# haliphinx/TCE-RVOS

Hardware: AMD Instinct MI355X
Metric: clips/s (T=5, 360×640, Swin-T) at 1/2/4/8 MI355X; mask IoU vs ref (higher is better)
Workload: dtype f32 (3xf16-split MFMA, f32 accumulate); 1 GPU; swin_t_p4w7 T=5 360x640 + 32-token text, B=1 clip per forward, flags --with_box_refine --binary --f_token 8 --qtrans (BASELINE config 2); clips_in_flight_per_gpu=1, clips_per_forward=1, same_clip_in_group=False, ranks_per_gpu=1, parallelism=clip-sharded x1

## Files before the change

include/tce_rvos.h:

```cpp
#ifndef TCE_RVOS_H
#define TCE_RVOS_H
#include <stdint.h>

#ifdef __cplusplus
extern "C" {
#endif

typedef void* tceStream;

int tce_abi_version(void);
const char* tce_last_error(void);

typedef struct {
  const float* A;
  const float* A2;
  const float* W;
  const float* bias;
  const float* res;
  float* C;
  int32_t M, N, K;
  int32_t lda, lda2, ldw, ldc, ldres;
  int32_t act, res_mode;
  int32_t batch;
  int64_t sA, sA2, sW, sBias, sC, sRes;
// ... 96 lines not shown
int tce_copy_segments(const tceCopySeg* segs, int32_t n, tceStream stream);
int tce_box_refine_f32(const float* tmp, const float* ref, float* out, int32_t n, int32_t ref_dim, tceStream stream);

int tce_mask_pack_f32(const float* params, float* w0f, float* tail, int32_t nl, int32_t T, int32_t Q, int32_t Cm,
                      tceStream stream);
int tce_mask_tail_f32(const float* G, const float* tail, const float* refs , int32_t ref_ld,
                      float* masks, int32_t nl, int32_t T, int32_t Q, int32_t h, int32_t w, float img_h, float img_w,
                      int32_t stride_px, tceStream stream);

int tce_select_masks_u8(const float* logits, const float* masks, uint8_t* out, int32_t* best_query, int32_t T,
                        int32_t Q, int32_t K, int32_t h, int32_t w, int32_t H0, int32_t W0, float threshold,
                        tceStream stream);

int tce_resize_h_u8(const uint8_t* in, const int32_t* coef, const int32_t* bounds, uint8_t* tmp, int64_t rows,
                    int32_t Win, int32_t Wout, int32_t ksize, tceStream stream);
int tce_resize_v_norm_f32(const uint8_t* tmp, const int32_t* coef, const int32_t* bounds, const float* lut, float* out,
                          int32_t T, int32_t Hin, int32_t W, int32_t Hout, int32_t ksize, tceStream stream);

int tce_embed_ln_f32(const int64_t* ids, const int64_t* pos_ids, const float* word, const float* pos, const float* type0,
                     const float* gamma, const float* beta, float* out, int32_t L, int32_t C, float eps, int32_t pad_id,
                     tceStream stream);
int tce_embed_ln_seqs_f32(const int64_t* ids, const float* word, const float* pos, const float* type0, const float* gamma,
                          const float* beta, float* out, int32_t nseq, int32_t seq_len, int32_t C, float eps, int32_t pad_id,
                          tceStream stream);
int tce_mha_small64_f32(const float* qkv, float* out, int32_t L, int32_t nheads, float scale, tceStream stream);
int tce_tanh_f32(const float* x, float* out, int64_t n, tceStream stream);

int32_t tce_thin_linear_splits(int32_t M, int32_t N, int32_t K);
int tce_thin_partials_f32(const float* x, int64_t ldx, int32_t xsplits, const float* bias_x, int32_t act_x, const float* W,
                          int64_t ldw, float* ws, int32_t M, int32_t N, int32_t K, tceStream stream);
int tce_splitk_reduce_f32(const float* ws, int32_t splits, int32_t M, int32_t N, const float* bias, int32_t act, const float* res,
                          int32_t ldres, int32_t res_mode, float* C, int32_t ldc, const float* gamma, const float* beta, float eps,
                          tceStream stream);
int tce_mha_small64_splits_f32(const float* qkv_planes, int32_t splits, const float* bias, float* out, int32_t L, int32_t nheads,
                               float scale, tceStream stream);
int tce_mha_small64_seqs_f32(const float* qkv_planes, int32_t splits, const float* bias, float* out, int32_t nseq, int32_t L,
                             int32_t nheads, float scale, tceStream stream);
int tce_mha_small64_lens_f32(const float* qkv_planes, int32_t splits, const float* bias, float* out, int32_t nseq, int32_t L,
                             int32_t nheads, float scale, const int32_t* lens, tceStream stream);
int tce_caption_lens_f32(const int64_t* ids, int32_t nseq, int32_t Lmax, int32_t pad_id, int32_t D, int32_t* lens, uint8_t* kmask,
                         float* pos, tceStream stream);

int64_t tce_ffn_packed_bytes(int32_t C, int32_t Hd);
int tce_ffn_pack_f32(const float* W1, const float* b1, const float* W2, void* packed, int32_t C, int32_t Hd,
                     tceStream stream);
int tce_ffn_pack_batched_f32(const float* W1, const float* b1, const float* W2, void* packed, int32_t C, int32_t Hd,
                             int32_t batch, tceStream stream);
int tce_ffn_fused_f32(const float* x, int64_t ldx, const void* packed, const float* b2, const float* g_in,
                      const float* be_in, float eps_in, const float* g_out, const float* be_out, float eps_out,
                      float* out, int64_t ldo, int32_t M, int32_t C, int32_t Hd, int32_t act, tceStream stream);
int64_t tce_ffn_split_ws_floats(int32_t M, int32_t C, int32_t Hd, int32_t act);
int32_t tce_ffn_split_counters(int32_t M, int32_t C, int32_t Hd, int32_t act);
int tce_ffn_fused_split_f32(const float* x, int64_t ldx, const void* packed, const float* b2, const float* g_in, const float* be_in,
                            float eps_in, const float* g_out, const float* be_out, float eps_out, float* out, int64_t ldo, int32_t M,
                            int32_t C, int32_t Hd, int32_t act, float* ws, int64_t ws_floats, int32_t* counters, int32_t n_counters,
                            tceStream stream);

typedef struct {
  const float* x;
  const float* a2;
  const void* packed;
  const float* bias;
  const float* res;
  float* out;
  const float *g_in, *be_in, *g_out, *be_out;
  int64_t ldx, lda2, ldres, ldo;
  int64_t sX, sA2, sRes, sOut;
  int32_t M, N, K, batch, a2_rows, act, res_mode;
  float eps_in, eps_out;
} tceRowLinArgs;
int64_t tce_rowlin_packed_bytes(int32_t N, int32_t K);
int tce_rowlin_pack_f32(const float* W, int64_t ldw, void* packed, int32_t N, int32_t K, tceStream stream);
int tce_rowlin_f32(const tceRowLinArgs* args, tceStream stream);

int64_t tce_conv3x3_packed_bytes(int32_t Cin, int32_t N);
int tce_conv3x3_pack_f32(const float* w, void* packed, int32_t Cin, int32_t N, tceStream stream);
int tce_conv3x3_f32(const float* x, int64_t ldx, const void* packed, const float* bias, float* out, int64_t ldo, int32_t T,
                    int32_t H, int32_t W, int32_t Cin, int32_t N, tceStream stream);
int64_t tce_conv3x3_split_ws_floats(int32_t M, int32_t Cin, int32_t N);
int32_t tce_conv3x3_split_pieces(int32_t M, int32_t Cin, int32_t N);
int32_t tce_conv3x3_split_kstep(int32_t pieces, int32_t s);
int tce_conv3x3_split_f32(const float* x, int64_t ldx, const void* packed, const float* bias, float* out, int64_t ldo, int32_t T,
                          int32_t H, int32_t W, int32_t Cin, int32_t N, float* ws, int64_t ws_floats, tceStream stream);

typedef struct {
  const float* x;
  const float* a2;
  const void* packed;
  const float* bo;
  const float* res;
  float* out;
  const float *g_out, *be_out;
  int64_t ldx, lda2, ldres, ldo;
  int64_t sX, sRes, sOut, sW;
  int32_t M, batch, a2_rows, res_mode, group;
  float eps_out;
  int32_t w_div;
} tceXattnArgs;
int tce_xattn_prepare_f32(const float* k, const float* v, const float* wqT_ext, const float* wo, float* W1, float* b1,
                          float* W2, int32_t L, int32_t group, int32_t batch, tceStream stream);
int tce_xattn_fused_f32(const tceXattnArgs* args, tceStream stream);

typedef struct {
  const void* packed;
  const float* b2;
  const float* g_out;
  const float* be_out;
  float* mid;
  int64_t ldmid, sMid;
  int32_t hidden, act;
  float eps_out;
} tceXattnFfnArgs;
int tce_ffn_pack_chain_f32(const float* W1, const float* b1, const float* W2, void* packed, int32_t C, int32_t Hd, tceStream stream);
int tce_xattn_ffn_fused_f32(const tceXattnArgs* args, const tceXattnFfnArgs* ffn, tceStream stream);
int tce_xattn_pack_f32(const float* k, const float* v, const float* wqT_ext, const float* wo, void* packed, int32_t L, int32_t group,
                       int32_t batch, tceStream stream);
int tce_xattn_prepare_lens_f32(const float* k, const float* v, const float* wqT_ext, const float* wo, float* W1, float* b1, float* W2,
                               int32_t L, int32_t group, int32_t batch, const int32_t* lens, tceStream stream);
int tce_xattn_pack_lens_f32(const float* k, const float* v, const float* wqT_ext, const float* wo, void* packed, int32_t L,
                            int32_t group, int32_t batch, const int32_t* lens, tceStream stream);

int64_t tce_swin_attn_packed_bytes(int32_t C);
int tce_swin_attn_pack_f32(const float* Wqkv, const float* Wproj, void* packed, int32_t C, tceStream stream);
int tce_swin_attn_fused_f32(const float* x, int64_t ldx, const void* packed, const float* qkv_bias, const float* proj_bias,
                            const float* bias_table, const float* gamma1, const float* beta1, float eps, float* out, int64_t ldo,
                            int32_t T, int32_t H, int32_t W, int32_t C, int32_t shift, tceStream stream);

int tce_graph_begin(tceStream stream);
int tce_graph_end(tceStream stream, void** graph_exec_out);
int tce_graph_launch(void* graph_exec, tceStream stream);
int tce_graph_destroy(void* graph_exec);
int tce_graph_group(void* const* graphs, int32_t n, void** graph_exec_out);

typedef struct {
  const float* W;
  const float* bias;
  float* out;
  int32_t N, ldw, ldo;
  int32_t use_a2;
  int32_t act;
} tceFewRowSeg;
typedef struct {
  const float* x;
  const float* a2;
  const float* res;
  int64_t ldx, lda2, ldres;
  int32_t a2_rows, R, K, nseg;
  tceFewRowSeg seg[3];
  const float* g_in;
  const float* be_in;
  float* xn_out;
  int64_t ldxn;
  float eps_in;
} tceFewRowArgs;
int tce_fewrow_linear_f32(const tceFewRowArgs* args, tceStream stream);

#ifdef __cplusplus
}
#endif
#endif
```

tce-rvos_amd/_lib.py:

```python
import ctypes as C
import os

HERE = os.path.dirname(os.path.abspath(__file__))
LIB_PATH = os.environ.get("TCE_LIB") or os.path.join(HERE, "lib", "libtce_rvos.so")

c_f = C.c_void_p
i32, i64, f32 = C.c_int32, C.c_int64, C.c_float


class GemmArgs(C.Structure):
    _fields_ = [("A", c_f), ("A2", c_f), ("W", c_f), ("bias", c_f), ("res", c_f), ("C", c_f),
                ("M", i32), ("N", i32), ("K", i32),
                ("lda", i32), ("lda2", i32), ("ldw", i32), ("ldc", i32), ("ldres", i32),
                ("act", i32), ("res_mode", i32), ("batch", i32),
                ("sA", i64), ("sA2", i64), ("sW", i64), ("sBias", i64), ("sC", i64), ("sRes", i64),
                ("conv", i32), ("T", i32), ("H", i32), ("Wd", i32), ("Cin", i32), ("Ho", i32), ("Wo", i32),
                ("kh", i32), ("kw", i32), ("stride", i32), ("pad", i32)]


class RowLinArgs(C.Structure):
    _fields_ = [("x", c_f), ("a2", c_f), ("packed", c_f), ("bias", c_f), ("res", c_f), ("out", c_f),
                ("g_in", c_f), ("be_in", c_f), ("g_out", c_f), ("be_out", c_f),
                ("ldx", i64), ("lda2", i64), ("ldres", i64), ("ldo", i64),
                ("sX", i64), ("sA2", i64), ("sRes", i64), ("sOut", i64),
# ... 29 lines not shown
class CopySeg(C.Structure):
    _fields_ = [("src", c_f), ("dst", c_f), ("rows", i64), ("row_words", i64), ("src_pitch_words", i64)]


SIGNATURES = {
    "tce_abi_version": (i32, []),
    "tce_last_error": (C.c_char_p, []),
    "tce_gemm_f32": (i32, [C.POINTER(GemmArgs), c_f]),
    "tce_gemm_splitk_f32": (i32, [C.POINTER(GemmArgs), i32, c_f, c_f]),
    "tce_gemm_splitk_ln_f32": (i32, [C.POINTER(GemmArgs), i32, c_f, c_f, c_f, f32, c_f]),
    "tce_gemm_select_tile": (i32, [i32, i32, i32]),
    "tce_gemm_select_tile_ex": (i32, [i32, i32, i32, i32, i32]),
    "tce_set_gemm_mode": (i32, [i32]),
    "tce_set_gemm_mode_thread": (i32, [i32]),
    "tce_set_range_flag": (i32, [c_f]),
    "tce_get_gemm_mode": (i32, []),
    "tce_layernorm_f32": (i32, [c_f, c_f, c_f, c_f, c_f, i64, i32, f32, c_f]),
    "tce_groupnorm_nsplit": (i32, [i32]),
    "tce_groupnorm_f32": (i32, [c_f, c_f, c_f, c_f, c_f, i32, i32, i32, i32, f32, i32, c_f]),
    "tce_groupnorm_up_add_f32": (i32, [c_f, c_f, c_f, c_f, c_f, c_f, i32, i32, i32, i32, i32, i32, i32, f32, i32, c_f]),
    "tce_resnet_stem_f32": (i32, [c_f, c_f, c_f, c_f, i32, i32, i32, c_f]),
    "tce_maxpool3x3s2_cl_f32": (i32, [c_f, c_f, i32, i32, i32, i32, c_f]),
    "tce_resize_h_u8": (i32, [c_f, c_f, c_f, c_f, i64, i32, i32, i32, c_f]),
    "tce_resize_v_norm_f32": (i32, [c_f, c_f, c_f, c_f, c_f, i32, i32, i32, i32, i32, c_f]),
    "tce_patch_embed_f32": (i32, [c_f, c_f, c_f, c_f, c_f, c_f, i32, i32, i32, i32, f32, c_f]),
    "tce_window_attn_f32": (i32, [c_f, c_f, c_f, c_f, i32, i32, i32, i32, i32, i32, c_f]),
    "tce_window_attn3d_f32": (i32, [c_f, c_f, c_f, c_f, i32, i32, i32, i32, i32, i32, c_f]),
    "tce_patch_merge_ln_f32": (i32, [c_f, c_f, c_f, c_f, i32, i32, i32, i32, f32, c_f]),
    "tce_mha_f32": (i32, [c_f, c_f, c_f, c_f, i32, i32, i32, i32, i32, i32, i32, i32, i64, i64, i64, i64, c_f, f32, c_f]),
    "tce_mha_ws_bytes": (i64, [i32, i32, i32]),
    "tce_mha_ws_f32": (i32, [c_f, c_f, c_f, c_f, c_f, i32, i32, i32, i32, i32, i32, i32, i32, i64, i64, i64, i64, c_f, f32, c_f]),
    "tce_ms_deform_attn_forward_f32": (i32, [c_f, c_f, c_f, c_f, c_f, c_f, i32, i32, i32, i32, i32, i32, i32, c_f]),
    "tce_ms_deform_attn_backward_f32": (i32, [c_f, c_f, c_f, c_f, c_f, c_f, c_f, c_f, c_f, i32, i32, i32, i32, i32, i32, i32, c_f]),
    "tce_msda_fused_f32": (i32, [c_f, c_f, c_f, c_f, C.POINTER(i32), i32, i32, i32, i32, i32, i32, i32, i32, c_f]),
    "tce_msda_fused_valid_f32": (i32, [c_f, c_f, c_f, c_f, C.POINTER(i32), C.POINTER(i32), i32, i32, i32, i32, i32, i32, i32,
                                       i32, c_f]),
    "tce_msda_fewq_raw_f32": (i32, [c_f, c_f, c_f, c_f, c_f, c_f, C.POINTER(i32), C.POINTER(i32), i32, i32, i32, i32, i32, i32, i32,
                                    i32, c_f]),
    "tce_contrastive_f32": (i32, [c_f, c_f, c_f, c_f, i32, i32, i32, i32, c_f]),
    "tce_pos_sine2d_f32": (i32, [c_f, c_f, i32, i32, i32, i32, c_f]),
    "tce_pos_sine2d_valid_f32": (i32, [c_f, c_f, i32, i32, i32, i32, i32, i32, c_f]),
    "tce_resize_nearest_f32": (i32, [c_f, c_f, c_f, i32, i32, i32, i32, i32, i32, c_f]),
    "tce_resize_bilinear_f32": (i32, [c_f, c_f, c_f, i32, i32, i32, i32, i32, i32, c_f]),
    "tce_resize_bilinear_ln_f32": (i32, [c_f, c_f, c_f, c_f, f32, c_f, i32, i32, i32, i32, i32, i32, c_f]),
    "tce_add_f32": (i32, [c_f, c_f, c_f, i64, i64, c_f]),
    "tce_tile_f32": (i32, [c_f, c_f, i64, i64, c_f]),
    "tce_sigmoid_f32": (i32, [c_f, c_f, i64, c_f]),
    "tce_copy_segments": (i32, [C.POINTER(CopySeg), i32, c_f]),
    "tce_box_refine_f32": (i32, [c_f, c_f, c_f, i32, i32, c_f]),
    "tce_mask_pack_f32": (i32, [c_f, c_f, c_f, i32, i32, i32, i32, c_f]),
    "tce_mask_tail_f32": (i32, [c_f, c_f, c_f, i32, c_f, i32, i32, i32, i32, i32, f32, f32, i32, c_f]),
    "tce_select_masks_u8": (i32, [c_f, c_f, c_f, c_f, i32, i32, i32, i32, i32, i32, i32, f32, c_f]),
    "tce_embed_ln_f32": (i32, [c_f, c_f, c_f, c_f, c_f, c_f, c_f, c_f, i32, i32, f32, i32, c_f]),
    "tce_mha_small64_f32": (i32, [c_f, c_f, i32, i32, f32, c_f]),
    "tce_mha_small64_seqs_f32": (i32, [c_f, i32, c_f, c_f, i32, i32, i32, f32, c_f]),
    "tce_embed_ln_seqs_f32": (i32, [c_f, c_f, c_f, c_f, c_f, c_f, c_f, i32, i32, i32, f32, i32, c_f]),
    "tce_mha_small64_lens_f32": (i32, [c_f, i32, c_f, c_f, i32, i32, i32, f32, c_f, c_f]),
    "tce_caption_lens_f32": (i32, [c_f, i32, i32, i32, i32, c_f, c_f, c_f, c_f]),
    "tce_tanh_f32": (i32, [c_f, c_f, i64, c_f]),
    "tce_ffn_packed_bytes": (i64, [i32, i32]),
    "tce_ffn_pack_f32": (i32, [c_f, c_f, c_f, c_f, i32, i32, c_f]),
    "tce_ffn_fused_f32": (i32, [c_f, i64, c_f, c_f, c_f, c_f, f32, c_f, c_f, f32, c_f, i64, i32, i32, i32, i32, c_f]),
    "tce_ffn_split_ws_floats": (i64, [i32, i32, i32, i32]),
    "tce_ffn_split_counters": (i32, [i32, i32, i32, i32]),
    "tce_ffn_fused_split_f32": (i32, [c_f, i64, c_f, c_f, c_f, c_f, f32, c_f, c_f, f32, c_f, i64, i32, i32, i32, i32, c_f, i64, c_f, i32, c_f]),
    "tce_xattn_prepare_f32": (i32, [c_f, c_f, c_f, c_f, c_f, c_f, c_f, i32, i32, i32, c_f]),
    "tce_ffn_pack_batched_f32": (i32, [c_f, c_f, c_f, c_f, i32, i32, i32, c_f]),
    "tce_xattn_fused_f32": (i32, [C.POINTER(XattnArgs), c_f]),
    "tce_xattn_ffn_fused_f32": (i32, [C.POINTER(XattnArgs), C.POINTER(XattnFfnArgs), c_f]),
    "tce_ffn_pack_chain_f32": (i32, [c_f, c_f, c_f, c_f, i32, i32, c_f]),
    "tce_xattn_pack_f32": (i32, [c_f, c_f, c_f, c_f, c_f, i32, i32, i32, c_f]),
    "tce_xattn_prepare_lens_f32": (i32, [c_f, c_f, c_f, c_f, c_f, c_f, c_f, i32, i32, i32, c_f, c_f]),
    "tce_xattn_pack_lens_f32": (i32, [c_f, c_f, c_f, c_f, c_f, i32, i32, i32, c_f, c_f]),
    "tce_rowlin_packed_bytes": (i64, [i32, i32]),
    "tce_rowlin_pack_f32": (i32, [c_f, i64, c_f, i32, i32, c_f]),
    "tce_rowlin_f32": (i32, [C.POINTER(RowLinArgs), c_f]),
    "tce_conv3x3_packed_bytes": (i64, [i32, i32]),
    "tce_conv3x3_pack_f32": (i32, [c_f, c_f, i32, i32, c_f]),
    "tce_conv3x3_f32": (i32, [c_f, i64, c_f, c_f, c_f, i64, i32, i32, i32, i32, i32, c_f]),
    "tce_conv3x3_split_ws_floats": (i64, [i32, i32, i32]),
    "tce_conv3x3_split_pieces": (i32, [i32, i32, i32]),
    "tce_conv3x3_split_kstep": (i32, [i32, i32]),
    "tce_conv3x3_split_f32": (i32, [c_f, i64, c_f, c_f, c_f, i64, i32, i32, i32, i32, i32, c_f, i64, c_f]),
    "tce_fewrow_linear_f32": (i32, [C.POINTER(FewRowArgs), c_f]),
    "tce_thin_linear_splits": (i32, [i32, i32, i32]),
    "tce_thin_partials_f32": (i32, [c_f, i64, i32, c_f, i32, c_f, i64, c_f, i32, i32, i32, c_f]),
    "tce_splitk_reduce_f32": (i32, [c_f, i32, i32, i32, c_f, i32, c_f, i32, i32, c_f, i32, c_f, c_f, f32, c_f]),
    "tce_mha_small64_splits_f32": (i32, [c_f, i32, c_f, c_f, i32, i32, f32, c_f]),
    "tce_swin_attn_packed_bytes": (i64, [i32]),
    "tce_swin_attn_pack_f32": (i32, [c_f, c_f, c_f, i32, c_f]),
    "tce_swin_attn_fused_f32": (i32, [c_f, i64, c_f, c_f, c_f, c_f, c_f, c_f, f32, c_f, i64, i32, i32, i32, i32, i32, c_f]),
    "tce_graph_begin": (i32, [c_f]),
    "tce_graph_end": (i32, [c_f, C.POINTER(C.c_void_p)]),
    "tce_graph_launch": (i32, [C.c_void_p, c_f]),
    "tce_graph_destroy": (i32, [C.c_void_p]),
    "tce_graph_group": (i32, [C.POINTER(C.c_void_p), i32, C.POINTER(C.c_void_p)]),
}

DEBUG_SIGNATURES = {
    "tce_gemm_force_tile": (i32, [i32]),
    "tce_debug_set_stamp_buffer": (i32, [c_f]),
    "tce_debug_set_epilogue": (i32, [i32]),
    "tce_debug_ffn_set_stamp_buffer": (i32, [c_f]),
    "tce_debug_ffn_set_half": (i32, [i32]),
    "tce_debug_msda_set_lds": (i32, [i32]),
    "tce_debug_window_attn_set_mfma": (i32, [i32]),
    "tce_debug_mha_set_split": (i32, [i32]),
    "tce_debug_msda_set_fewq": (i32, [i32]),
    "tce_debug_conv3x3_set_waves": (i32, [i32]),
    "tce_debug_conv3x3_set_pieces": (i32, [i32]),
}

_LIB = None


class TceError(RuntimeError):
    pass


def lib():
    global _LIB
    if _LIB is None:
        if not os.path.exists(LIB_PATH):
            raise TceError(f"{LIB_PATH} not found: build the HIP extension first "
                           f"(python -c 'import __graft_entry__ as g; g.build()'); there is no fallback path")
        hwq = os.environ.get("GPU_MAX_HW_QUEUES")
        if hwq not in (None, "", "4"):
            import warnings
            warnings.warn(f"tce_rvos_amd: GPU_MAX_HW_QUEUES={hwq} is set; the HIP runtime's default (4) is the only value this "
                          f"launch program runs well with (1-3 crash the runtime, 5-16 double the clip time)", RuntimeWarning)
        l = C.CDLL(LIB_PATH)
        for name, (res, args) in list(SIGNATURES.items()) + list(DEBUG_SIGNATURES.items()):
            fn = getattr(l, name)
            fn.restype = res
            fn.argtypes = args
        _LIB = l
    return _LIB


def lib_raw():
    l = lib()
    return l.__dict__.get("_real", l)


def check(status, what=""):
    if status != 0:
        msg = lib().tce_last_error().decode(errors="replace")
        raise TceError(f"{what} failed ({status}): {msg}")
```

tce-rvos_amd/build.py:

```python
import glob
import os
from concurrent.futures import ThreadPoolExecutor
import subprocess
import sys

HERE = os.path.dirname(os.path.abspath(__file__))
CSRC = os.path.join(HERE, "csrc")
OBJ = os.path.join(CSRC, "_obj")
LIBDIR = os.path.join(HERE, "lib")
LIB = os.path.join(LIBDIR, "libtce_rvos.so")
SOURCES = ["gemm_f16x3_big_256_split.hip", "gemm_f16x3_big_256_single.hip", "gemm_f16x3_big_128_split.hip", "gemm_f16x3_big_128_single.hip",
           "chain_ffn.hip", "chain_rowlin.hip", "gemm_f16x3_big.hip", "gemm_f16x3_small.hip", "gemm.hip", "attn.hip", "misc.hip", "norm.hip", "msda.hip",
           "text.hip", "resnet.hip", "frontend.hip", "fewrow.hip", "swinattn.hip", "thin.hip", "capi.hip"]
HIPCC = os.environ.get("HIPCC", "/opt/rocm/bin/hipcc")
FLAGS = ["--offload-arch=gfx950", "-O3", "-fPIC", "-std=c++17", "-Wall", "-Wno-unused-function"] + \
    os.environ.get("HIPCC_EXTRA", "").split()


def _newer(src_list, target):
    if not os.path.exists(target):
        return True
    t = os.path.getmtime(target)
    return any(os.path.getmtime(s) > t for s in src_list)


def build(verbose=True, force=False):
    os.makedirs(OBJ, exist_ok=True)
    os.makedirs(LIBDIR, exist_ok=True)
    headers = sorted(glob.glob(os.path.join(CSRC, "*.h")) + glob.glob(os.path.join(CSRC, "*.inc"))) + [os.path.join(HERE, "..", "include", "tce_rvos.h"),
                                                             os.path.join(CSRC, "chain.hip")]
    objs, todo = [], []
    for s in SOURCES:
        src = os.path.join(CSRC, s)
        obj = os.path.join(OBJ, s.replace(".hip", ".o"))
        if force or _newer([src] + headers, obj):
            todo.append([HIPCC] + FLAGS + ["-c", src, "-o", obj])
        objs.append(obj)

    def run(cmd):
        if verbose:
            print(" ".join(cmd), flush=True)
        subprocess.check_call(cmd)

    jobs = int(os.environ.get("TCE_BUILD_JOBS", min(8, os.cpu_count() or 1)))
    with ThreadPoolExecutor(max_workers=max(1, jobs)) as pool:
        list(pool.map(run, todo))
    if force or _newer(objs, LIB):
        tmp = LIB + f".tmp{os.getpid()}"
        cmd = [HIPCC, "--offload-arch=gfx950", "-shared", "-fPIC", "-o", tmp] + objs
        if verbose:
            print(" ".join(cmd), flush=True)
        subprocess.check_call(cmd)
        os.replace(tmp, LIB)
    return LIB


if __name__ == "__main__":
    print(build(force="--force" in sys.argv))
```

tce-rvos_amd/csrc/chain.hip:

```cpp
#include "common.h"
#include "gemm_epilogue.h"
#include "frag.h"
#include "../../include/tce_rvos.h"
#include "../../include/tce_rvos_debug.h"

namespace {

#ifndef FFN_ABL
#define FFN_ABL 0
#endif
static __device__ long long* g_ffn_stamps = nullptr;


template <int K, bool HAS_A2 = true>
__device__ __forceinline__ void load_x_frags(const float* __restrict__ x, const long long ldx,
                                             const float* __restrict__ a2, const long long lda2, const int a2_rows,
                                             const int m0, const int M, float* __restrict__ wt, const int lane,
                                             const float* __restrict__ g_in, const float* __restrict__ be_in,
                                             const float eps, h16x8 (&xh)[K / 16], h16x8 (&xl)[K / 16],
                                             const int single = 0) {
  constexpr int NP = K / 32;
  const int cr = lane >> 3, cp = (lane & 7) * 4;
  const int r = lane & 31, hf = lane >> 5;
  f32x4 v[NP][4];
// ... 996 lines not shown
  const int Hd = 8 * G, NC = Hd / 32;
  const int Lb = lens ? min(lens[blockIdx.y], L) : L;
  k += (long long)blockIdx.y * L * C;
  v += (long long)blockIdx.y * L * C;
  out += (long long)blockIdx.y * units * 16;
  const int lane = (int)(tix & 63);
  const long long sg = tix >> 6;
  const int sl = (int)(sg % SL), it = (int)(sg / SL);
  const int r = lane & 31, hf = lane >> 5;
  u32x4* const stage_out = reinterpret_cast<u32x4*>(out) + (long long)it * P * 64;
  auto dot32 = [](const float* a, const float* b) {
    const f32x4* ap = reinterpret_cast<const f32x4*>(a);
    const f32x4* bp = reinterpret_cast<const f32x4*>(b);
    float acc = 0.f;
#pragma unroll
    for (int c4 = 0; c4 < 8; ++c4) {
      const f32x4 x = ap[c4], y = bp[c4];
      acc = fmaf(x[0], y[0], acc); acc = fmaf(x[1], y[1], acc); acc = fmaf(x[2], y[2], acc); acc = fmaf(x[3], y[3], acc);
    }
    return acc;
  };
  if (sl == 0) {
    u32x4 o = {0u, 0u, 0u, 0u};
    if (lane < 8 && it < NC) {
      f32x4 val;
#pragma unroll
      for (int c = 0; c < 4; ++c) {
        const int idx = 4 * lane + c, h2 = idx >> 4, i = idx & 15;
        const int row = 32 * it + (i & 3) + 8 * (i >> 2) + 4 * h2, h = row / G, j = row - h * G;
        float a = -1.0e30f;
        if (j < Lb) {
          a = 0.f;
          for (int c2 = 0; c2 < HD; ++c2) a = fmaf(k[j * C + h * HD + c2], wqT[(long long)C * C + h * HD + c2], a);
        }
        val[c] = a;
      }
      o = __builtin_bit_cast(u32x4, val);
    }
    stage_out[lane] = o;
    return;
  }
  const int p_hi = 2 * sl - 1, p_lo = 2 * sl;
  if (p_hi >= P) return;
  u32x4 oh = {0u, 0u, 0u, 0u}, ol = oh;
  if (p_hi < 1 + 2 * KS + 4 * NT) {
    float val[8];
    if (p_hi <= 2 * KS) {
      const int s = (p_hi - 1) >> 1;
      const int row = 32 * it + r, h = row / G, j = row - h * G;
#pragma unroll
      for (int e = 0; e < 8; ++e)
        val[e] = (it < NC && j < Lb) ? dot32(k + j * C + h * HD, wqT + (long long)(16 * s + 8 * hf + e) * C + h * HD) : 0.f;
    } else {
      const int idx = (p_hi - 1 - 2 * KS) >> 1, t = idx >> 1, s2 = idx & 1, chunk = it - 1;
#pragma unroll
      for (int e = 0; e < 8; ++e) {
        const int col = 32 * chunk + 16 * s2 + 8 * (e >> 2) + 4 * hf + (e & 3);
        const int h = col / G, j = col - h * G;
        val[e] = (chunk >= 0 && chunk < NC && j < Lb) ? dot32(wo + (long long)(32 * t + r) * C + h * HD, v + j * C + h * HD) : 0.f;
      }
    }
    const HL f = split8(val, single);
    oh = __builtin_bit_cast(u32x4, f.hi);
    ol = __builtin_bit_cast(u32x4, f.lo);
  }
  stage_out[p_hi * 64 + lane] = oh;
  if (p_lo < P) stage_out[p_lo * 64 + lane] = ol;
}

constexpr int CONV_PAD_STAGES = 6;

struct ConvArgs {
  const float* x;
  const unsigned char* wpk;
  const float* bias;
  float* out;
  long long ldx, ldo;
  int H, W, M;
  int* range_flag;
  int single;
  int m_off;
  int nb, pieces;
  float* ws;
};

constexpr int CONV_ITERS = 12;
__host__ __device__ constexpr int conv3x3_piece_iter(const int pieces, const int s) { return s * CONV_ITERS / pieces; }

#ifndef CONV_ABL
#define CONV_ABL 0
#endif

template <int BYTE_OFF>
__device__ __forceinline__ void gload16(f32x4& dst, const float* ptr) {
  asm volatile("global_load_dwordx4 %0, %1, off offset:%2" : "=v"(dst) : "v"(ptr), "n"(BYTE_OFF) : "memory");
}

template <int I, int N, typename F>
__device__ __forceinline__ void static_for(F&& f) {
  if constexpr (I < N) {
    f(std::integral_constant<int, I>{});
    static_for<I + 1, N>(f);
  }
}

template <int CIN, bool SINGLE, int WAVES = 4, bool SPLIT = false>
__global__ void __launch_bounds__(64 * WAVES, WAVES / 4) conv3x3_kernel(const ConvArgs p) {
  constexpr int NTL = 8;
  constexpr int PW = 16 / WAVES;
  constexpr int STAGE = 2 * NTL * PIECE;
  constexpr int R = 4;
  constexpr int XS = WAVES == 4 ? 6 : 4, LX = XS + 1;
  constexpr int NW = WAVES == 4 ? CONV_PAD_STAGES - 2 : 3, LW = NW + 2;
  constexpr int INFLIGHT = (2 + PW) * (LW - 3);
  static_assert(LW <= CONV_PAD_STAGES, "the packed stream's zero padding covers the weight lead");
  constexpr int BODY = 12;
  constexpr int ITERS = 3 * (CIN / 64);
  constexpr int KS = BODY * ITERS;
  static_assert(CIN % 64 == 0, "channel chunks come in groups of four");
  static_assert(BODY % R == 0 && BODY % XS == 0 && BODY % NW == 0 && LX >= LW, "ring positions are compile-time");
  static_assert(WAVES * WT_BYTES <= R * STAGE, "the epilogue's staging tiles alias the ring");
  static_assert(!SPLIT || (ITERS == CONV_ITERS && WAVES == 4 && !SINGLE), "split pieces: CIN = 256, 128-pixel workgroups, split fp16");
  __shared__ __attribute__((aligned(16))) unsigned char smem[R * STAGE];

  const int tid = threadIdx.x, lane = tid & 63;
  const int wave = __builtin_amdgcn_readfirstlane(tid >> 6);
  const int hf = lane >> 5;
  const int blk = SPLIT ? (int)blockIdx.x % p.nb : (int)blockIdx.x;
  const int piece = SPLIT ? (int)blockIdx.x / p.nb : 0;
  const int i0 = SPLIT ? conv3x3_piece_iter(p.pieces, piece) : 0;
  const int i1 = SPLIT ? conv3x3_piece_iter(p.pieces, piece + 1) : ITERS;
  const int m0 = p.m_off + blk * (32 * WAVES) + wave * 32;

  const int m = m0 + (lane & 31);
  const int px = m % p.W, py = (m / p.W) % p.H;
  const float* const zeros = reinterpret_cast<const float*>(p.wpk + (long long)(KS + CONV_PAD_STAGES) * STAGE) + 8 * hf;
  const float* const xme = p.x + (long long)min(m, p.M - 1) * p.ldx + 8 * hf;
  auto iter_ptrs = [&](const int it, const float* (&q)[3]) {
    const int dy = it / (CIN / 64) - 1, cq = it % (CIN / 64);
    const bool row_ok = it < i1 && m < p.M && (unsigned)(py + dy) < (unsigned)p.H;
#pragma unroll
    for (int d = 0; d < 3; ++d) {
      const bool ok = row_ok && (unsigned)(px + d - 1) < (unsigned)p.W;
      q[d] = (ok ? xme + (long long)(dy * p.W + d - 1) * p.ldx : zeros) + 64 * cq;
    }
  };

  const float* wp = reinterpret_cast<const float*>(p.wpk + ((long long)i0 * BODY * STAGE) + (long long)(PW * wave) * PIECE + lane * 16);
  unsigned char* const wdst = smem + (PW * wave) * PIECE + lane * 16;
  f32x4 wr[NW][PW];
  auto wload = [&](f32x4 (&dst)[PW]) {
    if (!(CONV_ABL & 8)) {
      gload16<0>(dst[0], wp);
      gload16<PIECE>(dst[1], wp);
      if constexpr (PW == 4) {
        gload16<2 * PIECE>(dst[2], wp);
        gload16<3 * PIECE>(dst[3], wp);
      }
    }
    wp += STAGE / 4;
  };
  auto wstore = [&](const f32x4 (&src)[PW], const int stage) {
#pragma unroll
    for (int q = 0; q < PW; ++q) *reinterpret_cast<f32x4*>(wdst + stage * STAGE + q * PIECE) = src[q];
  };

  f32x4 xr[XS][2];
  const float* cur[3];
  const float* nxt[3];
  iter_ptrs(i0, cur);
  iter_ptrs(i0 + 1, nxt);
  auto xload = [&](auto jjc, f32x4 (&dst)[2]) {
    constexpr int JJ = decltype(jjc)::value;
    constexpr int J = JJ % BODY;
    const float* const src = JJ < BODY ? cur[J % 3] : nxt[J % 3];
    if (CONV_ABL & 16) return;
    gload16<64 * (J / 3)>(dst[0], src);
    gload16<64 * (J / 3) + 16>(dst[1], src);
  };
  auto wait_loads = [&](auto nc, f32x4 (&xs)[2], f32x4 (&ws)[PW]) {
    constexpr int N = (CONV_ABL & 24) ? 0 : decltype(nc)::value;
    if constexpr (PW == 4) {
      asm volatile("s_waitcnt vmcnt(%6)"
                   : "+v"(xs[0]), "+v"(xs[1]), "+v"(ws[0]), "+v"(ws[1]), "+v"(ws[2]), "+v"(ws[3])
                   : "n"(N)
                   : "memory");
    } else {
      asm volatile("s_waitcnt vmcnt(%4)" : "+v"(xs[0]), "+v"(xs[1]), "+v"(ws[0]), "+v"(ws[1]) : "n"(N) : "memory");
    }
  };
  using nfl = std::integral_constant<int, INFLIGHT>;

  f32x16 acc[NTL];
#pragma unroll
  for (int t = 0; t < NTL; ++t)
#pragma unroll
    for (int i = 0; i < 16; ++i) acc[t][i] = 0.f;
  h16x8 bh, bl;
  static_for<0, LX>([&](auto mc) {
    constexpr int m = decltype(mc)::value - LX;
    if constexpr (m + 2 >= 0) {
      wait_loads(nfl{}, xr[(m + 2) % XS], wr[(m + 2) % NW]);
      wstore(wr[(m + 2) % NW], (m + 2) % R);
      if constexpr (m + 2 == 0) {
        const float f[8] = {xr[0][0][0], xr[0][0][1], xr[0][0][2], xr[0][0][3], xr[0][1][0], xr[0][1][1], xr[0][1][2], xr[0][1][3]};
        const HL b = split8(f, SINGLE ? 1 : 0);
        bh = b.hi;
        bl = b.lo;
        asm volatile("" : "+v"(bh), "+v"(bl));
      }
    }
    if constexpr (m + LX >= 0) xload(std::integral_constant<int, m + LX>{}, xr[(m + LX) % XS]);
    if constexpr (m + LW >= 0) wload(wr[(m + LW) % NW]);
  });
  __syncthreads();
  h16x8 fh[4], fl[4];
  {
    const unsigned char* const st = smem + lane * 16;
    fh[0] = *reinterpret_cast<const h16x8*>(st);
    fl[0] = *reinterpret_cast<const h16x8*>(st + PIECE);
    fh[1] = *reinterpret_cast<const h16x8*>(st + 2 * PIECE);
    fl[1] = *reinterpret_cast<const h16x8*>(st + 3 * PIECE);
  }

  for (int it = i0; it < i1; ++it) {
    static_for<0, BODY>([&](auto jc) {
      constexpr int j = decltype(jc)::value;
      constexpr int nslot = (j + 1) % XS;
      const unsigned char* const st = smem + (j % R) * STAGE + lane * 16;
      unsigned nh[4], nl[4];
      auto tile = [&](auto tc) {
        constexpr int t = decltype(tc)::value;
#if CONV_ABL & 4
        const h16x8 k0 = fh[t % 4], k1 = fl[t % 4], k2 = bh, k3 = bl;
        asm volatile("" : : "v"(k0), "v"(k1), "v"(k2), "v"(k3));
#else
        if constexpr (!SINGLE) {
          acc[t] = __builtin_amdgcn_mfma_f32_32x32x16_f16(fh[t % 4], bl, acc[t], 0, 0, 0);
          acc[t] = __builtin_amdgcn_mfma_f32_32x32x16_f16(fl[t % 4], bh, acc[t], 0, 0, 0);
        }
        acc[t] = __builtin_amdgcn_mfma_f32_32x32x16_f16(fh[t % 4], bh, acc[t], 0, 0, 0);
#endif
      };
      static_for<0, 6>([&](auto tc) {
        constexpr int t = decltype(tc)::value;
        fh[(t + 2) % 4] = *reinterpret_cast<const h16x8*>(st + (2 * t + 4) * PIECE);
        fl[(t + 2) % 4] = *reinterpret_cast<const h16x8*>(st + (2 * t + 5) * PIECE);
        __builtin_amdgcn_sched_barrier(0);
        tile(tc);
        if constexpr (t < 4) {
          const float a = xr[nslot][t >> 1][2 * (t & 1)], b = xr[nslot][t >> 1][2 * (t & 1) + 1];
          if constexpr (SINGLE) {
            nh[t] = __builtin_bit_cast(unsigned, fp16x2_t{(__fp16)a, (__fp16)b});
            nl[t] = 0u;
          } else {
            const fp16x2_t h = __builtin_amdgcn_cvt_pkrtz(a, b);
            nh[t] = __builtin_bit_cast(unsigned, h);
            nl[t] = __builtin_bit_cast(unsigned, __builtin_amdgcn_cvt_pkrtz(a - (float)h[0], b - (float)h[1]));
          }
          asm volatile("" : "+v"(nh[t]), "+v"(nl[t]));
        }
        __builtin_amdgcn_sched_barrier(0);
      });
      wait_loads(nfl{}, xr[(j + 2) % XS], wr[(j + 2) % NW]);
      wstore(wr[(j + 2) % NW], (j + 2) % R);
      if (!(CONV_ABL & 2)) __syncthreads();
      xload(std::integral_constant<int, j + LX>{}, xr[(j + LX) % XS]);
      wload(wr[(j + LW) % NW]);
      {
        const unsigned char* const sn = smem + ((j + 1) % R) * STAGE + lane * 16;
        fh[0] = *reinterpret_cast<const h16x8*>(sn);
        fl[0] = *reinterpret_cast<const h16x8*>(sn + PIECE);
        fh[1] = *reinterpret_cast<const h16x8*>(sn + 2 * PIECE);
        fl[1] = *reinterpret_cast<const h16x8*>(sn + 3 * PIECE);
      }
      __builtin_amdgcn_sched_barrier(0);
      tile(std::integral_constant<int, 6>{});
      tile(std::integral_constant<int, 7>{});
      __builtin_amdgcn_sched_barrier(0);
      bh = __builtin_bit_cast(h16x8, u32x4{nh[0], nh[1], nh[2], nh[3]});
      bl = __builtin_bit_cast(h16x8, u32x4{nl[0], nl[1], nl[2], nl[3]});
    });
#pragma unroll
    for (int d = 0; d < 3; ++d) cur[d] = nxt[d];
    iter_ptrs(it + 2, nxt);
  }
  asm volatile("s_waitcnt vmcnt(0)" ::: "memory");
  __syncthreads();

  float* const wt = reinterpret_cast<float*>(smem + wave * WT_BYTES);
  tce_amax_t amax = 0;
  if constexpr (SPLIT) {
    float* const part = p.ws + (long long)piece * (p.M - p.m_off) * 256;
#pragma unroll
    for (int t = 0; t < NTL; ++t) tile_store(acc[t], part, 256, m0 - p.m_off, p.M - p.m_off, 32 * t, wt, lane, amax);
    return;
  }
  const ResTile none = {};
#pragma unroll
  for (int t = 0; t < NTL; ++t) {
    tile_bias_res<0>(acc[t], tile_bias_load(p.bias, 32 * t, lane), none, wt, lane);
    tile_store(acc[t], p.out, p.ldo, m0, p.M, 32 * t, wt, lane, amax);
  }
  tce_range_report(p.range_flag, amax);
}

__global__ void __launch_bounds__(256) conv3x3_reduce_kernel(const float* __restrict__ ws, const int pieces, const int rows,
                                                             const float* __restrict__ bias, float* __restrict__ out,
                                                             const long long ldo, const int m_off, int* range_flag) {
  const long long n4 = (long long)rows * 64, stride = (long long)gridDim.x * 256;
  tce_amax_t amax = 0;
  for (long long i = (long long)blockIdx.x * 256 + threadIdx.x; i < n4; i += stride) {
    const f32x4* src = reinterpret_cast<const f32x4*>(ws) + i;
    f32x4 v = src[0];
    for (int s = 1; s < pieces; ++s) v += src[(long long)s * n4];
    const int c4 = (int)(i & 63);
    if (bias) v += reinterpret_cast<const f32x4*>(bias)[c4];
    amax = tce_amax4(amax, v);
    *reinterpret_cast<f32x4*>(out + (m_off + (i >> 6)) * ldo + 4 * c4) = v;
  }
  tce_range_report(range_flag, amax);
}

__global__ void __launch_bounds__(256) conv3x3_pack_kernel(const float* __restrict__ w, unsigned char* __restrict__ out,
                                                           const int CIN, const long long units, const int single) {
  const long long u = (long long)blockIdx.x * 256 + threadIdx.x;
  if (u >= units) return;
  const int lane = (int)(u & 63);
  const long long pg = u >> 6;
  const int piece = (int)(pg & 15);
  const long long s = pg >> 4;
  const int r = lane & 31, hf = lane >> 5, t = piece >> 1;
  u32x4 o = {0u, 0u, 0u, 0u};
  if (s < 9 * CIN / 16) {
    const int it = (int)(s / 12), j = (int)(s % 12);
    const int dy = it / (CIN / 64), cc = 4 * (it % (CIN / 64)) + j / 3, dx = j % 3;
    float v[8];
#pragma unroll
    for (int e = 0; e < 8; ++e) v[e] = w[(long long)(32 * t + r) * (9 * CIN) + (3 * dy + dx) * CIN + 16 * cc + 8 * hf + e];
    const HL f = split8(v, single);
    o = __builtin_bit_cast(u32x4, (piece & 1) ? f.lo : f.hi);
  }
  reinterpret_cast<u32x4*>(out)[u] = o;
}

inline bool conv3x3_shape_ok(int Cin, int N) { return Cin == 256 && N == 256; }
inline long long conv3x3_units(int Cin) { return (long long)(9 * Cin / 16 + CONV_PAD_STAGES) * 16 * 64 + 128; }

template <int NT>
__global__ void __launch_bounds__(256) patch_embed_mfma_kernel(const float* __restrict__ frames, const float* __restrict__ w,
                                                               const float* __restrict__ b, const float* __restrict__ gamma,
                                                               const float* __restrict__ beta, float* __restrict__ out,
                                                               const int H, const int W, const float eps, const int ntok,
                                                               const int Hp, const int Wp, int* const range_flag,
                                                               const int single) {
  constexpr int C = 32 * NT;
  __shared__ __attribute__((aligned(16))) unsigned char wtbuf[4 * WT_BYTES];
  const int tid = threadIdx.x, lane = tid & 63;
  const int wave = __builtin_amdgcn_readfirstlane(tid >> 6);
  const int r = lane & 31, hf = lane >> 5;
  const int m0 = blockIdx.x * 128 + wave * 32;
  if (m0 >= ntok) return;
  float* const wt = reinterpret_cast<float*>(wtbuf + wave * WT_BYTES);

  const int tok = min(m0 + r, ntok - 1);
  const int t = tok / (Hp * Wp), rem = tok - t * (Hp * Wp);
  const int py = rem / Wp, px = rem - py * Wp;
  const bool vec = ((W & 3) == 0) && (px * 4 + 3 < W);
  f32x4 raw[3][2];
#pragma unroll
  for (int c = 0; c < 3; ++c)
#pragma unroll
    for (int q = 0; q < 2; ++q) {
      const int yy = py * 4 + 2 * hf + q;
      const float* const row = frames + (((long long)t * 3 + c) * H + min(yy, H - 1)) * W;
      f32x4 v = {0.f, 0.f, 0.f, 0.f};
      if (yy < H) {
        if (vec) {
          v = *reinterpret_cast<const f32x4*>(row + px * 4);
        } else {
#pragma unroll
          for (int kx = 0; kx < 4; ++kx)
            if (px * 4 + kx < W) v[kx] = row[px * 4 + kx];
        }
      }
      raw[c][q] = v;
    }
  h16x8 ah[NT][3], al[NT][3];
#pragma unroll
  for (int tt = 0; tt < NT; ++tt)
#pragma unroll
    for (int sK = 0; sK < 3; ++sK) {
      const float* const pw = w + (long long)(32 * tt + r) * 48 + 16 * sK + 8 * hf;
      const f32x4 a = *reinterpret_cast<const f32x4*>(pw), c4 = *reinterpret_cast<const f32x4*>(pw + 4);
      const float f[8] = {a[0], a[1], a[2], a[3], c4[0], c4[1], c4[2], c4[3]};
      const HL sp = split8(f, single);
      ah[tt][sK] = sp.hi;
      al[tt][sK] = sp.lo;
    }
  f32x16 acc[NT];
#pragma unroll
  for (int tt = 0; tt < NT; ++tt)
#pragma unroll
    for (int i = 0; i < 16; ++i) acc[tt][i] = 0.f;
#pragma unroll
  for (int sK = 0; sK < 3; ++sK) {
    const float f[8] = {raw[sK][0][0], raw[sK][0][1], raw[sK][0][2], raw[sK][0][3],
                        raw[sK][1][0], raw[sK][1][1], raw[sK][1][2], raw[sK][1][3]};
    const HL x = split8(f, single);
#pragma unroll
    for (int tt = 0; tt < NT; ++tt) {
      if (!single) {
        acc[tt] = __builtin_amdgcn_mfma_f32_32x32x16_f16(ah[tt][sK], x.lo, acc[tt], 0, 0, 0);
        acc[tt] = __builtin_amdgcn_mfma_f32_32x32x16_f16(al[tt][sK], x.hi, acc[tt], 0, 0, 0);
      }
      acc[tt] = __builtin_amdgcn_mfma_f32_32x32x16_f16(ah[tt][sK], x.hi, acc[tt], 0, 0, 0);
    }
  }
  const ResTile none = {};
#pragma unroll
  for (int tt = 0; tt < NT; ++tt) tile_bias_res<0>(acc[tt], tile_bias_load(b, 32 * tt, lane), none, wt, lane);
  rows_layernorm<NT>(acc, gamma, beta, eps, hf);
  tce_amax_t amax = 0;
#pragma unroll
  for (int tt = 0; tt < NT; ++tt) tile_store(acc[tt], out, C, m0, ntok, 32 * tt, wt, lane, amax);
  tce_range_report(range_flag, amax);
}

}

#ifndef TCE_CHAIN_PART
#define TCE_CHAIN_PART 0
#endif
int tce_chain_rowlin_set_stamps(long long* dev_buf);

#if TCE_CHAIN_PART != 2
extern "C" int tce_debug_ffn_set_stamp_buffer(long long* dev_buf) {
#if TCE_CHAIN_PART == 1
  if (tce_chain_rowlin_set_stamps(dev_buf) != 0) return -1;
#endif
  return hipMemcpyToSymbol(HIP_SYMBOL(g_ffn_stamps), &dev_buf, sizeof(dev_buf)) == hipSuccess ? 0 : -1;
}

extern "C" int64_t tce_ffn_packed_bytes(int32_t C, int32_t Hd) { return ffn_shape_ok(C, Hd) ? ffn_units(C, Hd) * 16 : -1; }

extern "C" int tce_ffn_pack_f32(const float* W1, const float* b1, const float* W2, void* packed, int32_t C, int32_t Hd,
                                tceStream stream) {
  TCE_CHECK_ARG(ffn_shape_ok(C, Hd), "tce_ffn_pack_f32: unsupported shape C=%d hidden=%d (C in 96/128/192/256, hidden %% 32 == 0)",
                C, Hd);
  TCE_CHECK_ARG(W1 && W2 && packed && tce_aligned16(packed), "tce_ffn_pack_f32: null / misaligned pointer");
  const long long units = ffn_units(C, Hd);
  hipLaunchKernelGGL(ffn_pack_kernel, dim3(tce_cdiv(units, 256)), dim3(256), 0, (hipStream_t)stream, W1, b1, W2,
                     (unsigned char*)packed, C, Hd, ffn_pieces(C), units, tce_gemm_single_pass());
  TCE_CHECK_LAUNCH("tce_ffn_pack_f32");
  return TCE_OK;
}

extern "C" int tce_ffn_pack_batched_f32(const float* W1, const float* b1, const float* W2, void* packed, int32_t C, int32_t Hd,
                                        int32_t batch, tceStream stream) {
  TCE_CHECK_ARG(ffn_shape_ok(C, Hd) && batch > 0, "tce_ffn_pack_batched_f32: unsupported shape C=%d hidden=%d batch=%d", C, Hd, batch);
  TCE_CHECK_ARG(W1 && W2 && packed && tce_aligned16(packed), "tce_ffn_pack_batched_f32: null / misaligned pointer");
  const long long units = ffn_units(C, Hd);
  hipLaunchKernelGGL(ffn_pack_kernel, dim3(tce_cdiv(units, 256), batch), dim3(256), 0, (hipStream_t)stream, W1, b1, W2,
                     (unsigned char*)packed, C, Hd, ffn_pieces(C), units, tce_gemm_single_pass());
  TCE_CHECK_LAUNCH("tce_ffn_pack_batched_f32");
  return TCE_OK;
}

extern "C" int tce_ffn_pack_chain_f32(const float* W1, const float* b1, const float* W2, void* packed, int32_t C, int32_t Hd,
                                      tceStream stream) {
  TCE_CHECK_ARG(C == 256 && ffn_shape_ok(C, Hd), "tce_ffn_pack_chain_f32: C must be 256, hidden %% 32 == 0 (C=%d hidden=%d)", C, Hd);
  TCE_CHECK_ARG(W1 && W2 && packed && tce_aligned16(packed), "tce_ffn_pack_chain_f32: null / misaligned pointer");
  const long long units = ffn_units(C, Hd);
  hipLaunchKernelGGL(ffn_pack_kernel, dim3(tce_cdiv(units, 256)), dim3(256), 0, (hipStream_t)stream, W1, b1, W2,
                     (unsigned char*)packed, C, Hd, ffn_pieces(C), units, tce_gemm_single_pass(), 1);
  TCE_CHECK_LAUNCH("tce_ffn_pack_chain_f32");
  return TCE_OK;
}

extern "C" int tce_ffn_fused_f32(const float* x, int64_t ldx, const void* packed, const float* b2, const float* g_in,
                                 const float* be_in, float eps_in, const float* g_out, const float* be_out,
                                 float eps_out, float* out, int64_t ldo, int32_t M, int32_t C, int32_t Hd, int32_t act,
                                 tceStream stream) {
  TCE_CHECK_ARG(ffn_shape_ok(C, Hd), "tce_ffn_fused_f32: unsupported shape C=%d hidden=%d", C, Hd);
  TCE_CHECK_ARG(M > 0 && x && packed && b2 && out, "tce_ffn_fused_f32: null pointer or M <= 0");
  TCE_CHECK_ARG(act == 1 || act == 2, "tce_ffn_fused_f32: act must be 1 (ReLU) or 2 (GELU)");
  TCE_CHECK_ARG(ldx >= C && ldo >= C && ldx % 4 == 0 && ldo % 4 == 0, "tce_ffn_fused_f32: bad row pitch");
  TCE_CHECK_ARG(tce_aligned16(x) && tce_aligned16(out) && tce_aligned16(packed) && tce_aligned16(b2),
                "tce_ffn_fused_f32: x/out/packed/b2 must be 16-byte aligned");
  TCE_CHECK_ARG((!g_in || (be_in && tce_aligned16(g_in) && tce_aligned16(be_in))) &&
                    (!g_out || (be_out && tce_aligned16(g_out) && tce_aligned16(be_out))),
                "tce_ffn_fused_f32: LayerNorm gamma/beta must come in pairs, 16-byte aligned");
  FfnArgs a = {};
  a.x = x; a.wpk = (const unsigned char*)packed; a.b2 = b2; a.res_mode = 1;
  a.g_in = g_in; a.be_in = be_in; a.g_out = g_out; a.be_out = be_out;
  a.out = out; a.ldx = ldx; a.ldo = ldo; a.M = M; a.NI = Hd / 32 + 1; a.eps_in = eps_in; a.eps_out = eps_out; a.range_flag = tce_range_flag(); a.single = tce_gemm_single_pass();
  a.wdiv = 1;
  hipStream_t s = (hipStream_t)stream;
  if (C == 256) ffn_launch<256, 4>(a, act, s);
  else if (C == 192) ffn_launch<192, 4>(a, act, s);
  else if (C == 128) ffn_launch<128, 8>(a, act, s);
  else ffn_launch<96, 8>(a, act, s);
  TCE_CHECK_LAUNCH("tce_ffn_fused_f32");
  return TCE_OK;
}

extern "C" int tce_debug_ffn_set_half(int32_t mode) {
  TCE_CHECK_ARG(mode >= -1 && mode <= 1, "tce_debug_ffn_set_half: -1 (never), 0 (automatic) or 1 (always)");
  g_ffn_half = mode;
  return TCE_OK;
}

extern "C" int64_t tce_ffn_split_ws_floats(int32_t M, int32_t C, int32_t Hd, int32_t act) {
  if (M <= 0 || !ffn_shape_ok(C, Hd) || act != 1) return 0;
  return ffn_split_plan(M, C, Hd, 1).ws_floats;
}

extern "C" int32_t tce_ffn_split_counters(int32_t M, int32_t C, int32_t Hd, int32_t act) {
  if (M <= 0 || !ffn_shape_ok(C, Hd) || act != 1) return 0;
// ... 79 lines not shown
extern "C" int tce_xattn_pack_lens_f32(const float* k, const float* v, const float* wqT_ext, const float* wo, void* packed, int32_t L,
                                       int32_t group, int32_t batch, const int32_t* lens, tceStream stream) {
  TCE_CHECK_ARG(k && v && wqT_ext && wo && packed && lens, "tce_xattn_pack_lens_f32: null pointer");
  TCE_CHECK_ARG((group == 32 || group == 8) && L > 0 && L <= group && batch > 0,
                "tce_xattn_pack_lens_f32: group must be 32 or 8, 0 < L <= group");
  TCE_CHECK_ARG(tce_aligned16(k) && tce_aligned16(v) && tce_aligned16(wqT_ext) && tce_aligned16(wo) && tce_aligned16(packed),
                "tce_xattn_pack_lens_f32: pointers must be 16-byte aligned");
  const int Hd = 8 * group;
  const long long units = ffn_units(256, Hd);
  const int P = ffn_pieces(256), SL = 1 + P / 2;
  const long long threads = (long long)(Hd / 32 + 2) * SL * 64;
  hipLaunchKernelGGL(xattn_pack_fused_kernel, dim3(tce_cdiv(threads, 256), batch), dim3(256), 0, (hipStream_t)stream, k, v, wqT_ext,
                     wo, (unsigned char*)packed, L, group, P, SL, threads, units, tce_gemm_single_pass(), (const int*)lens);
  TCE_CHECK_LAUNCH("tce_xattn_pack_lens_f32");
  return TCE_OK;
}

static int xattn_launch(const tceXattnArgs* args, const tceXattnFfnArgs* ffn, tceStream stream);

extern "C" int tce_xattn_fused_f32(const tceXattnArgs* args, tceStream stream) { return xattn_launch(args, nullptr, stream); }

extern "C" int tce_xattn_ffn_fused_f32(const tceXattnArgs* args, const tceXattnFfnArgs* ffn, tceStream stream) {
  TCE_CHECK_ARG(args && ffn, "tce_xattn_ffn_fused_f32: null args");
  TCE_CHECK_ARG(ffn->packed && ffn->b2 && ffn->mid && ffn->hidden > 0 && ffn->hidden % 32 == 0 && ffn_shape_ok(256, ffn->hidden),
                "tce_xattn_ffn_fused_f32: bad FFN stage (packed / b2 / mid / hidden)");
  TCE_CHECK_ARG(ffn->act == 1, "tce_xattn_ffn_fused_f32: the FFN stage's activation must be 1 (ReLU)");
  TCE_CHECK_ARG(ffn->ldmid >= 256 && ffn->ldmid % 4 == 0 && ffn->sMid % 4 == 0 && tce_aligned16(ffn->mid) && tce_aligned16(ffn->packed) &&
                    tce_aligned16(ffn->b2) && (!ffn->g_out || (ffn->be_out && tce_aligned16(ffn->g_out) && tce_aligned16(ffn->be_out))),
                "tce_xattn_ffn_fused_f32: FFN stage pitch / alignment");
  TCE_CHECK_ARG(args->res_mode == 1, "tce_xattn_ffn_fused_f32: the attention stage's residual must be additive");
  TCE_CHECK_ARG(ffn->mid != args->x && ffn->mid != args->out && ffn->mid != args->res,
                "tce_xattn_ffn_fused_f32: mid must be a buffer of its own (it is written and re-read inside the launch)");
  return xattn_launch(args, ffn, stream);
}

static int xattn_launch(const tceXattnArgs* args, const tceXattnFfnArgs* ffn, tceStream stream) {
  TCE_CHECK_ARG(args != nullptr, "tce_xattn_fused_f32: null args");
  const tceXattnArgs& q = *args;
  TCE_CHECK_ARG(q.M > 0 && q.x && q.packed && q.bo && q.out, "tce_xattn_fused_f32: null pointer or M <= 0");
  TCE_CHECK_ARG(q.res_mode == 1 || q.res_mode == 2, "tce_xattn_fused_f32: res_mode must be 1 (add) or 2 (multiply)");
  TCE_CHECK_ARG(q.group == 32 || q.group == 8, "tce_xattn_fused_f32: group (key slots per head) must be 32 or 8");
  TCE_CHECK_ARG(q.ldx >= 256 && q.ldo >= 256 && q.ldx % 4 == 0 && q.ldo % 4 == 0 && (!q.res || (q.ldres >= 256 && q.ldres % 4 == 0)) &&
                    (!q.a2 || (q.lda2 >= 256 && q.lda2 % 4 == 0)) && q.sX % 4 == 0 && q.sRes % 4 == 0 && q.sOut % 4 == 0,
                "tce_xattn_fused_f32: bad row pitch / batch stride");
  TCE_CHECK_ARG(tce_aligned16(q.x) && tce_aligned16(q.out) && tce_aligned16(q.packed) && tce_aligned16(q.bo) &&
                    (!q.a2 || tce_aligned16(q.a2)) && (!q.res || tce_aligned16(q.res)),
                "tce_xattn_fused_f32: pointers must be 16-byte aligned");
  TCE_CHECK_ARG(!q.g_out || (q.be_out && tce_aligned16(q.g_out) && tce_aligned16(q.be_out)),
                "tce_xattn_fused_f32: LayerNorm gamma/beta must come in pairs, 16-byte aligned");
  FfnArgs a = {};
  a.x = q.x; a.wpk = (const unsigned char*)q.packed; a.b2 = q.bo; a.g_out = q.g_out; a.be_out = q.be_out; a.out = q.out;
  a.ldx = q.ldx; a.ldo = q.ldo; a.a2 = q.a2; a.lda2 = q.lda2; a.a2_rows = q.a2_rows; a.res = q.res; a.ldres = q.ldres;
  a.res_mode = q.res_mode; a.sX = q.sX; a.sRes = q.sRes; a.sOut = q.sOut; a.sW = q.sW;
  a.M = q.M; a.NI = (8 * q.group) / 32 + 1; a.eps_out = q.eps_out; a.range_flag = tce_range_flag(); a.single = tce_gemm_single_pass();
  a.wdiv = q.w_div > 0 ? q.w_div : 1;
  const int batch = q.batch > 0 ? q.batch : 1;
  const dim3 grid(tce_cdiv(a.M, 128), batch), block(256);
  if (ffn) {
    a.wpk2 = (const unsigned char*)ffn->packed; a.b22 = ffn->b2; a.g_out2 = ffn->g_out; a.be_out2 = ffn->be_out; a.eps_out2 = ffn->eps_out;
    a.mid = ffn->mid; a.ldmid = ffn->ldmid; a.sMid = ffn->sMid; a.NI2 = ffn->hidden / 32 + 1;
    if (a.single) {
      if (q.group == 32) hipLaunchKernelGGL((ffn_fused_kernel<256, 4, 3, true, 1>), grid, block, 0, (hipStream_t)stream, a);
      else hipLaunchKernelGGL((ffn_fused_kernel<256, 4, 4, true, 1>), grid, block, 0, (hipStream_t)stream, a);
    } else {
      if (q.group == 32) hipLaunchKernelGGL((ffn_fused_kernel<256, 4, 3, false, 1>), grid, block, 0, (hipStream_t)stream, a);
      else hipLaunchKernelGGL((ffn_fused_kernel<256, 4, 4, false, 1>), grid, block, 0, (hipStream_t)stream, a);
    }
    TCE_CHECK_LAUNCH("tce_xattn_ffn_fused_f32");
    return TCE_OK;
  }
  if (a.single) {
    if (q.group == 32) hipLaunchKernelGGL((ffn_fused_kernel<256, 4, 3, true>), grid, block, 0, (hipStream_t)stream, a);
    else hipLaunchKernelGGL((ffn_fused_kernel<256, 4, 4, true>), grid, block, 0, (hipStream_t)stream, a);
  } else {
    if (q.group == 32) hipLaunchKernelGGL((ffn_fused_kernel<256, 4, 3, false>), grid, block, 0, (hipStream_t)stream, a);
    else hipLaunchKernelGGL((ffn_fused_kernel<256, 4, 4, false>), grid, block, 0, (hipStream_t)stream, a);
  }
  TCE_CHECK_LAUNCH("tce_xattn_fused_f32");
  return TCE_OK;
}

#endif

#if TCE_CHAIN_PART != 1
int tce_chain_rowlin_set_stamps(long long* dev_buf) {
  return hipMemcpyToSymbol(HIP_SYMBOL(g_ffn_stamps), &dev_buf, sizeof(dev_buf)) == hipSuccess ? 0 : -1;
}

extern "C" int64_t tce_rowlin_packed_bytes(int32_t N, int32_t K) { return rowlin_shape_ok(N, K) ? rowlin_units(N, K) * 16 : -1; }

extern "C" int tce_rowlin_pack_f32(const float* W, int64_t ldw, void* packed, int32_t N, int32_t K, tceStream stream) {
  TCE_CHECK_ARG(rowlin_shape_ok(N, K), "tce_rowlin_pack_f32: unsupported shape N=%d K=%d (K in 96/128/192/256/384/512, N %% 32 == 0)", N, K);
  TCE_CHECK_ARG(W && packed && tce_aligned16(packed) && ldw >= K, "tce_rowlin_pack_f32: null / misaligned pointer or ldw < K");
  const long long units = rowlin_units(N, K);
  hipLaunchKernelGGL(rowlin_pack_kernel, dim3(tce_cdiv(units, 256)), dim3(256), 0, (hipStream_t)stream, W,
                     (unsigned char*)packed, N, K, (long long)ldw, units, tce_gemm_single_pass());
  TCE_CHECK_LAUNCH("tce_rowlin_pack_f32");
  return TCE_OK;
}

extern "C" int tce_rowlin_f32(const tceRowLinArgs* args, tceStream stream) {
  TCE_CHECK_ARG(args != nullptr, "tce_rowlin_f32: null args");
  const tceRowLinArgs& q = *args;
  TCE_CHECK_ARG(rowlin_shape_ok(q.N, q.K), "tce_rowlin_f32: unsupported shape N=%d K=%d", q.N, q.K);
  TCE_CHECK_ARG(q.M > 0 && q.x && q.packed && q.out, "tce_rowlin_f32: null pointer or M <= 0");
  TCE_CHECK_ARG(q.act >= 0 && q.act <= 2 && q.res_mode >= 0 && q.res_mode <= 2, "tce_rowlin_f32: bad act / res_mode");
  TCE_CHECK_ARG(q.res_mode == 0 || q.res, "tce_rowlin_f32: res_mode set without res");
  TCE_CHECK_ARG(q.ldx >= q.K && q.ldx % 4 == 0 && q.ldo >= q.N && q.ldo % 4 == 0 && (!q.res || (q.ldres >= q.N && q.ldres % 4 == 0)) &&
                    (!q.a2 || (q.lda2 >= q.K && q.lda2 % 4 == 0)),
                "tce_rowlin_f32: bad row pitch");
  TCE_CHECK_ARG(q.sX % 4 == 0 && q.sA2 % 4 == 0 && q.sRes % 4 == 0 && q.sOut % 4 == 0, "tce_rowlin_f32: batch strides must be multiples of 4 floats");
  TCE_CHECK_ARG(tce_aligned16(q.x) && tce_aligned16(q.out) && tce_aligned16(q.packed) && (!q.a2 || tce_aligned16(q.a2)) &&
                    (!q.res || tce_aligned16(q.res)) && (!q.bias || tce_aligned16(q.bias)),
                "tce_rowlin_f32: pointers must be 16-byte aligned");
  TCE_CHECK_ARG((!q.g_in || (q.be_in && tce_aligned16(q.g_in) && tce_aligned16(q.be_in))) &&
                    (!q.g_out || (q.be_out && tce_aligned16(q.g_out) && tce_aligned16(q.be_out))),
                "tce_rowlin_f32: LayerNorm gamma/beta must come in pairs, 16-byte aligned");
  TCE_CHECK_ARG(!q.g_out || (q.N == 256 && q.K <= 384), "tce_rowlin_f32: the output LayerNorm is built for N = 256, K <= 384");
  LinArgs a;
  a.x = q.x; a.a2 = q.a2; a.wpk = (const unsigned char*)q.packed; a.bias = q.bias; a.res = q.res; a.out = q.out;
  a.g_in = q.g_in; a.be_in = q.be_in; a.g_out = q.g_out; a.be_out = q.be_out;
  a.ldx = q.ldx; a.lda2 = q.lda2; a.ldres = q.ldres; a.ldo = q.ldo;
  a.sX = q.sX; a.sA2 = q.sA2; a.sRes = q.sRes; a.sOut = q.sOut;
  a.M = q.M; a.N = q.N; a.a2_rows = q.a2_rows; a.act = q.act; a.res_mode = q.res_mode;
  a.eps_in = q.eps_in; a.eps_out = q.eps_out; a.range_flag = tce_range_flag(); a.single = tce_gemm_single_pass();
  const int batch = q.batch > 0 ? q.batch : 1;
  const bool row = q.g_out != nullptr;
  hipStream_t s = (hipStream_t)stream;
  if (q.K == 512) rowlin_launch<512>(a, batch, row, s);
  else if (q.K == 384) rowlin_launch<384>(a, batch, row, s);
  else if (q.K == 256) rowlin_launch<256>(a, batch, row, s);
  else if (q.K == 192) rowlin_launch<192>(a, batch, row, s);
  else if (q.K == 128) rowlin_launch<128>(a, batch, row, s);
  else rowlin_launch<96>(a, batch, row, s);
  TCE_CHECK_LAUNCH("tce_rowlin_f32");
  return TCE_OK;
}

#endif

#if TCE_CHAIN_PART != 2
extern "C" int64_t tce_conv3x3_packed_bytes(int32_t Cin, int32_t N) { return conv3x3_shape_ok(Cin, N) ? conv3x3_units(Cin) * 16 : -1; }

extern "C" int tce_conv3x3_pack_f32(const float* w, void* packed, int32_t Cin, int32_t N, tceStream stream) {
  TCE_CHECK_ARG(conv3x3_shape_ok(Cin, N), "tce_conv3x3_pack_f32: unsupported shape Cin=%d N=%d (256 -> 256)", Cin, N);
  TCE_CHECK_ARG(w && packed && tce_aligned16(packed), "tce_conv3x3_pack_f32: null / misaligned pointer");
  const long long units = conv3x3_units(Cin);
  hipLaunchKernelGGL(conv3x3_pack_kernel, dim3(tce_cdiv(units, 256)), dim3(256), 0, (hipStream_t)stream, w,
                     (unsigned char*)packed, Cin, units, tce_gemm_single_pass());
  TCE_CHECK_LAUNCH("tce_conv3x3_pack_f32");
  return TCE_OK;
}

static int g_conv3_waves = 0;
extern "C" int tce_debug_conv3x3_set_waves(int32_t waves) {
  TCE_CHECK_ARG(waves == 0 || waves == 4 || waves == 8, "tce_debug_conv3x3_set_waves: 0 (automatic), 4 or 8");
  g_conv3_waves = waves;
  return TCE_OK;
}

struct Conv3Plan {
  int wide = 4;
  int full8 = 0;
  int m_narrow = 0;
  int nb = 0;
  int pieces = 1;
  long long ws_floats = 0;
};
inline Conv3Plan conv3x3_plan(const int M, const int cus, const int single, const int force_waves, const int split, const int force_pieces) {
  Conv3Plan pl;
  const int r4 = tce_cdiv(tce_cdiv(M, 128), cus), r8 = tce_cdiv(tce_cdiv(M, 256), cus);
  const int full8 = tce_cdiv(M, 256) / cus;
  const int rem_px = M - full8 * 256 * cus;
  const int mixed4 = 7 * full8 + 4 * tce_cdiv(tce_cdiv(rem_px, 128), cus);
  if (!force_waves && !single && full8 >= 1 && rem_px > 0 && mixed4 < 4 * r4 && mixed4 < 7 * r8) {
    pl.full8 = full8 * cus;
    pl.m_narrow = full8 * 256 * cus;
  } else {
    pl.wide = force_waves ? force_waves : (4 * r4 > 7 * r8 ? 8 : 4);
    if (single) pl.wide = 4;
    if (pl.wide == 8) return pl;
  }
  pl.nb = tce_cdiv(M - pl.m_narrow, 128);
  if (!split || single || pl.nb >= cus) return pl;
  const double OVH = 0.5, LAUNCH = 0.3, RED_BPI = 8.0 * (3u << 20);
  const long long px = M - pl.m_narrow;
  auto cost = [&](int p) {
    const double walk = (double)tce_cdiv((long long)pl.nb * p, cus) * (tce_cdiv(CONV_ITERS, p) + OVH);
    return p == 1 ? walk : walk + LAUNCH + (double)(p + 1) * px * 1024.0 / RED_BPI;
  };
  int best = 1;
  for (int p = 2; p <= 6; ++p)
    if ((long long)pl.nb * p <= 2ll * cus && cost(p) < cost(best)) best = p;
  if (force_pieces > 0) best = force_pieces;
  if (best > 1) {
    pl.pieces = best;
    pl.ws_floats = (long long)best * px * 256;
  }
  return pl;
}

static int g_conv3_pieces = 0;
extern "C" int tce_debug_conv3x3_set_pieces(int32_t pieces) {
  TCE_CHECK_ARG(pieces >= 0 && pieces <= CONV_ITERS, "tce_debug_conv3x3_set_pieces: 0 (automatic) .. 12");
  g_conv3_pieces = pieces;
  return TCE_OK;
}

static int conv3_force_waves() {
  static const int env_force = []() { const char* e = getenv("TCE_CONV3_WAVES"); return e ? atoi(e) : 0; }();
  return g_conv3_waves ? g_conv3_waves : env_force;
}

static Conv3Plan conv3x3_plan_for(const int M, const bool split) {
  return conv3x3_plan(M, tce_cu_count(), tce_gemm_single_pass(), conv3_force_waves(), split, g_conv3_pieces);
}

extern "C" int64_t tce_conv3x3_split_ws_floats(int32_t M, int32_t Cin, int32_t N) {
  return conv3x3_shape_ok(Cin, N) && M > 0 ? conv3x3_plan_for(M, true).ws_floats : 0;
}
extern "C" int32_t tce_conv3x3_split_pieces(int32_t M, int32_t Cin, int32_t N) {
  return conv3x3_shape_ok(Cin, N) && M > 0 ? conv3x3_plan_for(M, true).pieces : 0;
}
extern "C" int32_t tce_conv3x3_split_kstep(int32_t pieces, int32_t s) {
  return pieces >= 1 && pieces <= CONV_ITERS && s >= 0 && s <= pieces ? 12 * conv3x3_piece_iter(pieces, s) : -1;
}

static int conv3x3_launch(const float* x, int64_t ldx, const void* packed, const float* bias, float* out, int64_t ldo, int32_t T,
                          int32_t H, int32_t W, int32_t Cin, int32_t N, float* ws, int64_t ws_floats, const bool split, tceStream stream,
                          const char* name) {
  TCE_CHECK_ARG(conv3x3_shape_ok(Cin, N), "%s: unsupported shape Cin=%d N=%d (256 -> 256)", name, Cin, N);
  TCE_CHECK_ARG(x && packed && out && T > 0 && H > 0 && W > 0 && (long long)T * H * W < (1ll << 31),
                "%s: null pointer or bad sizes", name);
  TCE_CHECK_ARG(ldx >= Cin && ldx % 4 == 0 && ldo >= N && ldo % 4 == 0, "%s: bad row pitch", name);
  TCE_CHECK_ARG(tce_aligned16(x) && tce_aligned16(out) && tce_aligned16(packed) && (!bias || tce_aligned16(bias)),
                "%s: pointers must be 16-byte aligned", name);
  ConvArgs a;
  a.x = x; a.wpk = (const unsigned char*)packed; a.bias = bias; a.out = out;
  a.ldx = ldx; a.ldo = ldo; a.H = H; a.W = W; a.M = T * H * W;
  a.range_flag = tce_range_flag(); a.single = tce_gemm_single_pass();
  a.m_off = 0; a.nb = 0; a.pieces = 1; a.ws = nullptr;
  hipStream_t s = (hipStream_t)stream;
  const Conv3Plan pl = conv3x3_plan_for(a.M, split);
  if (pl.pieces > 1)
    TCE_CHECK_ARG(ws && tce_aligned16(ws) && ws_floats >= pl.ws_floats,
                  "%s: workspace of %lld floats needed (tce_conv3x3_split_ws_floats), %lld given", name, pl.ws_floats, (long long)ws_floats);
  if (pl.full8) hipLaunchKernelGGL((conv3x3_kernel<256, false, 8>), dim3(pl.full8), dim3(512), 0, s, a);
  a.m_off = pl.m_narrow;
  if (pl.wide == 8) hipLaunchKernelGGL((conv3x3_kernel<256, false, 8>), dim3(tce_cdiv(a.M, 256)), dim3(512), 0, s, a);
  else if (a.single) hipLaunchKernelGGL((conv3x3_kernel<256, true>), dim3(pl.nb), dim3(256), 0, s, a);
  else if (pl.pieces == 1) hipLaunchKernelGGL((conv3x3_kernel<256, false>), dim3(pl.nb), dim3(256), 0, s, a);
  else {
    a.nb = pl.nb; a.pieces = pl.pieces; a.ws = ws;
    hipLaunchKernelGGL((conv3x3_kernel<256, false, 4, true>), dim3(pl.nb * pl.pieces), dim3(256), 0, s, a);
    const int rows = a.M - a.m_off;
    hipLaunchKernelGGL(conv3x3_reduce_kernel, dim3(std::min(tce_cdiv((long long)rows * 64, 256), 8 * tce_cu_count())), dim3(256), 0, s,
                       (const float*)ws, pl.pieces, rows, bias, out, ldo, a.m_off, a.range_flag);
  }
  TCE_CHECK_LAUNCH(name);
  return TCE_OK;
}

extern "C" int tce_conv3x3_f32(const float* x, int64_t ldx, const void* packed, const float* bias, float* out, int64_t ldo,
                               int32_t T, int32_t H, int32_t W, int32_t Cin, int32_t N, tceStream stream) {
  return conv3x3_launch(x, ldx, packed, bias, out, ldo, T, H, W, Cin, N, nullptr, 0, false, stream, "tce_conv3x3_f32");
}

extern "C" int tce_conv3x3_split_f32(const float* x, int64_t ldx, const void* packed, const float* bias, float* out, int64_t ldo,
                                     int32_t T, int32_t H, int32_t W, int32_t Cin, int32_t N, float* ws, int64_t ws_floats,
                                     tceStream stream) {
  return conv3x3_launch(x, ldx, packed, bias, out, ldo, T, H, W, Cin, N, ws, ws_floats, true, stream, "tce_conv3x3_split_f32");
}

bool tce_patch_embed_mfma(const float* frames, const float* w, const float* b, const float* gamma, const float* beta,
                          float* out, int H, int W, int C, float eps, long long ntok, int Hp, int Wp, hipStream_t s) {
  if ((C != 96 && C != 128 && C != 192) || ntok >= (1ll << 31) || !tce_aligned16(frames) || !tce_aligned16(out) ||
      !tce_aligned16(w) || !tce_aligned16(b) || !tce_aligned16(gamma) || !tce_aligned16(beta))
    return false;
  const dim3 grid(tce_cdiv(ntok, 128)), block(256);
  int* const rf = tce_range_flag();
  const int single = tce_gemm_single_pass();
  if (C == 96) hipLaunchKernelGGL((patch_embed_mfma_kernel<3>), grid, block, 0, s, frames, w, b, gamma, beta, out, H, W, eps, (int)ntok, Hp, Wp, rf, single);
  else if (C == 128) hipLaunchKernelGGL((patch_embed_mfma_kernel<4>), grid, block, 0, s, frames, w, b, gamma, beta, out, H, W, eps, (int)ntok, Hp, Wp, rf, single);
  else hipLaunchKernelGGL((patch_embed_mfma_kernel<6>), grid, block, 0, s, frames, w, b, gamma, beta, out, H, W, eps, (int)ntok, Hp, Wp, rf, single);
  return true;
}
#endif
```

tce-rvos_amd/hazard.py:

```python
import contextlib
import traceback

import numpy as np
import torch

from . import _lib

F = 4


def strided(ptr, run_bytes, *dims):
    if not ptr or run_bytes <= 0 or any(c <= 0 for c, _ in dims):
        return np.zeros((0, 2), dtype=np.int64)
    starts = np.array([int(ptr)], dtype=np.int64)
    for count, stride in dims:
        if count == 1 or stride == 0:
            continue
        starts = (starts[:, None] + (np.arange(int(count), dtype=np.int64) * int(stride))[None, :]).reshape(-1)
    iv = np.stack([starts, starts + int(run_bytes)], 1)
    return merge(iv)


def dense(ptr, nbytes):
    return strided(ptr, int(nbytes))
# ... 262 lines not shown
                                      [dense(_p(a[3]), a[4] * ((a[5] - 1) // 2 + 1) * ((a[6] - 1) // 2 + 1) * 64 * F)]),
    "tce_maxpool3x3s2_cl_f32": lambda a: ([dense(_p(a[0]), a[2] * a[3] * a[4] * a[5] * F)],
                                          [dense(_p(a[1]), a[2] * ((a[3] - 1) // 2 + 1) * ((a[4] - 1) // 2 + 1) * a[5] * F)]),
    "tce_patch_embed_f32": lambda a: ([dense(_p(a[0]), a[6] * 3 * a[7] * a[8] * F), dense(_p(a[1]), a[9] * 48 * F)],
                                      [dense(_p(a[5]), a[6] * ((a[7] + 3) // 4) * ((a[8] + 3) // 4) * a[9] * F)]),
    "tce_window_attn_f32": _win,
    "tce_window_attn3d_f32": _win,
    "tce_patch_merge_ln_f32": lambda a: ([dense(_p(a[0]), a[4] * a[5] * a[6] * a[7] * F)],
                                         [dense(_p(a[3]), a[4] * ((a[5] + 1) // 2) * ((a[6] + 1) // 2) * 4 * a[7] * F)]),
    "tce_mha_f32": lambda a: _mha(a[0], a[1], a[2], a[3], None, *a[4:17]),
    "tce_mha_ws_f32": lambda a: _mha(a[0], a[1], a[2], a[3], a[4], *a[5:18]),
    "tce_ms_deform_attn_forward_f32": lambda a: (
        [dense(_p(a[0]), a[6] * a[7] * a[8] * a[9] * F), dense(_p(a[1]), a[11] * 16), dense(_p(a[2]), a[11] * 8),
         dense(_p(a[3]), a[6] * a[10] * a[8] * a[11] * a[12] * 2 * F), dense(_p(a[4]), a[6] * a[10] * a[8] * a[11] * a[12] * F)],
        [dense(_p(a[5]), a[6] * a[10] * a[8] * a[9] * F)]),
    "tce_ms_deform_attn_backward_f32": lambda a: (
        [dense(_p(a[0]), a[9] * a[10] * a[11] * a[12] * F), dense(_p(a[3]), a[9] * a[13] * a[11] * a[14] * a[15] * 2 * F),
         dense(_p(a[4]), a[9] * a[13] * a[11] * a[14] * a[15] * F), dense(_p(a[5]), a[9] * a[13] * a[11] * a[12] * F)],
        [dense(_p(a[6]), a[9] * a[10] * a[11] * a[12] * F), dense(_p(a[7]), a[9] * a[13] * a[11] * a[14] * a[15] * 2 * F),
         dense(_p(a[8]), a[9] * a[13] * a[11] * a[14] * a[15] * F)]),
    "tce_msda_fused_f32": lambda a: _msda(a[0], a[1], a[2], a[3], *a[5:13]),
    "tce_msda_fused_valid_f32": lambda a: _msda(a[0], a[1], a[2], a[3], *a[6:14]),
    "tce_msda_fewq_raw_f32": lambda a: (
        [dense(_p(a[0]), a[8] * a[9] * 256 * F), dense(_p(a[1]), 256 * 256 * F), dense(_p(a[2]), 256 * F),
         dense(_p(a[3]), a[8] * a[11] * a[10] * a[12] * a[13] * 3 * F), dense(_p(a[4]), (a[8] if a[15] else 1) * a[11] * a[14] * F)],
        [dense(_p(a[5]), a[8] * a[11] * 256 * F)]),
    "tce_contrastive_f32": lambda a: ([dense(_p(a[0]), a[4] * a[5] * a[6] * F), dense(_p(a[1]), (a[4] // a[7]) * a[6] * F)],
                                      [dense(_p(a[2]), a[4] * F), dense(_p(a[3]), a[4] * 32 * a[6] * F)]),
    "tce_pos_sine2d_f32": lambda a: _pos(a, False),
    "tce_pos_sine2d_valid_f32": lambda a: _pos(a, True),
    "tce_resize_nearest_f32": _resize,
    "tce_resize_bilinear_f32": _resize,
    "tce_resize_bilinear_ln_f32": _resize_ln,
    "tce_add_f32": lambda a: ([dense(_p(a[0]), a[3] * F), dense(_p(a[1]), a[4] * F)], [dense(_p(a[2]), a[3] * F)]),
    "tce_tile_f32": lambda a: ([dense(_p(a[0]), a[2] * F)], [dense(_p(a[1]), a[2] * a[3] * F)]),
    "tce_sigmoid_f32": lambda a: ([dense(_p(a[0]), a[2] * F)], [dense(_p(a[1]), a[2] * F)]),
    "tce_tanh_f32": lambda a: ([dense(_p(a[0]), a[2] * F)], [dense(_p(a[1]), a[2] * F)]),
    "tce_copy_segments": _copy_segments,
    "tce_box_refine_f32": lambda a: ([dense(_p(a[0]), a[3] * 4 * F), dense(_p(a[1]), a[3] * a[4] * F)], [dense(_p(a[2]), a[3] * 4 * F)]),
    "tce_mask_pack_f32": _mask_pack,
    "tce_mask_tail_f32": _mask_tail,
    "tce_select_masks_u8": lambda a: ([dense(_p(a[0]), a[4] * a[5] * a[6] * F), dense(_p(a[1]), a[4] * a[5] * a[7] * a[8] * F)],
                                      [dense(_p(a[2]), a[4] * a[9] * a[10]), dense(_p(a[3]), 4)]),
    "tce_resize_h_u8": lambda a: ([dense(_p(a[0]), a[4] * a[5] * 3)], [dense(_p(a[3]), a[4] * a[6] * 3)]),
    "tce_resize_v_norm_f32": lambda a: ([dense(_p(a[0]), a[5] * a[6] * a[7] * 3)], [dense(_p(a[4]), a[5] * 3 * a[8] * a[7] * F)]),
    "tce_embed_ln_f32": _embed,
    "tce_mha_small64_f32": lambda a: ([dense(_p(a[0]), a[2] * 3 * a[3] * 64 * F)], [dense(_p(a[1]), a[2] * a[3] * 64 * F)]),
    "tce_ffn_pack_f32": lambda a: _ffn_pack(a, False),
    "tce_ffn_pack_batched_f32": lambda a: _ffn_pack(a, True),
    "tce_ffn_fused_f32": _ffn_fused,
    "tce_ffn_fused_split_f32": _ffn_fused_split,
    "tce_xattn_prepare_f32": lambda a: (
        [dense(_p(a[0]), a[9] * a[7] * 256 * F), dense(_p(a[1]), a[9] * a[7] * 256 * F), dense(_p(a[2]), 257 * 256 * F),
         dense(_p(a[3]), 256 * 256 * F)],
        [dense(_p(a[4]), a[9] * 8 * a[8] * 256 * F), dense(_p(a[5]), a[9] * 8 * a[8] * F), dense(_p(a[6]), a[9] * 8 * a[8] * 256 * F)]),
    "tce_xattn_fused_f32": lambda a: _xattn(_st(a[0])),
    "tce_xattn_ffn_fused_f32": lambda a: _xattn_ffn(_st(a[0]), _st(a[1])),
    "tce_ffn_pack_chain_f32": lambda a: _ffn_pack(a, False),
    "tce_xattn_pack_f32": lambda a: (
        [dense(_p(a[0]), a[7] * a[5] * 256 * F), dense(_p(a[1]), a[7] * a[5] * 256 * F), dense(_p(a[2]), 257 * 256 * F), dense(_p(a[3]), 256 * 256 * F)],
        [dense(_p(a[4]), a[7] * _lib.lib_raw().tce_ffn_packed_bytes(256, 8 * a[6]))]),
    "tce_xattn_prepare_lens_f32": lambda a: (
        [dense(_p(a[0]), a[9] * a[7] * 256 * F), dense(_p(a[1]), a[9] * a[7] * 256 * F), dense(_p(a[2]), 257 * 256 * F),
         dense(_p(a[3]), 256 * 256 * F), dense(_p(a[10]), a[9] * 4)],
        [dense(_p(a[4]), a[9] * 8 * a[8] * 256 * F), dense(_p(a[5]), a[9] * 8 * a[8] * F), dense(_p(a[6]), a[9] * 8 * a[8] * 256 * F)]),
    "tce_xattn_pack_lens_f32": lambda a: (
        [dense(_p(a[0]), a[7] * a[5] * 256 * F), dense(_p(a[1]), a[7] * a[5] * 256 * F), dense(_p(a[2]), 257 * 256 * F), dense(_p(a[3]), 256 * 256 * F),
         dense(_p(a[8]), a[7] * 4)],
        [dense(_p(a[4]), a[7] * _lib.lib_raw().tce_ffn_packed_bytes(256, 8 * a[6]))]),
    "tce_rowlin_pack_f32": lambda a: ([strided(_p(a[0]), a[4] * F, (a[3], a[1] * F))],
                                      [dense(_p(a[2]), _lib.lib_raw().tce_rowlin_packed_bytes(a[3], a[4]))]),
    "tce_rowlin_f32": lambda a: _rowlin(_st(a[0])),
    "tce_conv3x3_pack_f32": lambda a: ([dense(_p(a[0]), a[3] * 9 * a[2] * F)],
                                       [dense(_p(a[1]), _lib.lib_raw().tce_conv3x3_packed_bytes(a[2], a[3]))]),
    "tce_conv3x3_f32": lambda a: (
        [strided(_p(a[0]), a[9] * F, (a[6] * a[7] * a[8], a[1] * F)), dense(_p(a[2]), _lib.lib_raw().tce_conv3x3_packed_bytes(a[9], a[10])),
         dense(_p(a[3]), a[10] * F)],
        [strided(_p(a[4]), a[10] * F, (a[6] * a[7] * a[8], a[5] * F))]),
    "tce_conv3x3_split_f32": lambda a: (
        [strided(_p(a[0]), a[9] * F, (a[6] * a[7] * a[8], a[1] * F)), dense(_p(a[2]), _lib.lib_raw().tce_conv3x3_packed_bytes(a[9], a[10])),
         dense(_p(a[3]), a[10] * F)],
        [strided(_p(a[4]), a[10] * F, (a[6] * a[7] * a[8], a[5] * F)),
         dense(_p(a[11]), _lib.lib_raw().tce_conv3x3_split_ws_floats(a[6] * a[7] * a[8], a[9], a[10]) * F)]),
    "tce_fewrow_linear_f32": lambda a: _fewrow(_st(a[0])),
    "tce_thin_partials_f32": lambda a: (
        [(strided(_p(a[0]), a[10] * F, (a[8], a[1] * F)) if a[2] == 0 else dense(_p(a[0]), a[2] * a[8] * a[10] * F)),
         dense(_p(a[3]), a[10] * F), strided(_p(a[5]), a[10] * F, (a[9], a[6] * F))],
        [dense(_p(a[7]), (a[10] // 256) * a[8] * a[9] * F)]),
    "tce_splitk_reduce_f32": lambda a: (
        [dense(_p(a[0]), a[1] * a[2] * a[3] * F), dense(_p(a[4]), a[3] * F), dense(_p(a[11]), a[3] * F), dense(_p(a[12]), a[3] * F)] +
        ([strided(_p(a[6]), a[3] * F, (a[2], a[7] * F))] if a[8] else []),
        [strided(_p(a[9]), a[3] * F, (a[2], a[10] * F))]),
    "tce_mha_small64_splits_f32": lambda a: ([dense(_p(a[0]), a[1] * a[4] * 3 * a[5] * 64 * F), dense(_p(a[2]), 3 * a[5] * 64 * F)],
                                             [dense(_p(a[3]), a[4] * a[5] * 64 * F)]),
    "tce_mha_small64_seqs_f32": lambda a: ([dense(_p(a[0]), a[1] * a[4] * a[5] * 3 * a[6] * 64 * F), dense(_p(a[2]), 3 * a[6] * 64 * F)],
                                           [dense(_p(a[3]), a[4] * a[5] * a[6] * 64 * F)]),
    "tce_mha_small64_lens_f32": lambda a: ([dense(_p(a[0]), a[1] * a[4] * a[5] * 3 * a[6] * 64 * F), dense(_p(a[2]), 3 * a[6] * 64 * F),
                                            dense(_p(a[8]), a[4] * 4)],
                                           [dense(_p(a[3]), a[4] * a[5] * a[6] * 64 * F)]),
    "tce_caption_lens_f32": lambda a: ([dense(_p(a[0]), a[1] * a[2] * 8)],
                                       [dense(_p(a[5]), a[1] * 4), dense(_p(a[6]), a[1] * a[2]), dense(_p(a[7]), a[1] * a[2] * a[4] * F)]),
    "tce_embed_ln_seqs_f32": lambda a: ([dense(_p(a[0]), a[7] * a[8] * 8), dense(_p(a[4]), a[9] * F), dense(_p(a[5]), a[9] * F)],
                                        [dense(_p(a[6]), a[7] * a[8] * a[9] * F)]),
    "tce_swin_attn_pack_f32": lambda a: ([dense(_p(a[0]), 3 * a[3] * a[3] * F), dense(_p(a[1]), a[3] * a[3] * F)],
                                         [dense(_p(a[2]), _lib.lib_raw().tce_swin_attn_packed_bytes(a[3]))]),
    "tce_swin_attn_fused_f32": lambda a: (
        [strided(_p(a[0]), a[14] * F, (a[11] * a[12] * a[13], a[1] * F)), dense(_p(a[2]), _lib.lib_raw().tce_swin_attn_packed_bytes(a[14])),
         dense(_p(a[3]), 3 * a[14] * F), dense(_p(a[4]), a[14] * F), dense(_p(a[5]), 169 * (a[14] // 32) * F),
         dense(_p(a[6]), a[14] * F), dense(_p(a[7]), a[14] * F)],
        [strided(_p(a[9]), a[14] * F, (a[11] * a[12] * a[13], a[10] * F))]),
}
NOT_LAUNCHES = {"tce_abi_version", "tce_last_error", "tce_gemm_select_tile", "tce_gemm_select_tile_ex", "tce_set_gemm_mode", "tce_set_gemm_mode_thread",
                "tce_get_gemm_mode", "tce_set_range_flag", "tce_groupnorm_nsplit", "tce_mha_ws_bytes", "tce_ffn_packed_bytes", "tce_ffn_split_ws_floats", "tce_ffn_split_counters",
                "tce_rowlin_packed_bytes", "tce_conv3x3_packed_bytes", "tce_conv3x3_split_ws_floats",
                "tce_conv3x3_split_pieces", "tce_conv3x3_split_kstep", "tce_swin_attn_packed_bytes", "tce_thin_linear_splits", "tce_graph_begin", "tce_graph_end", "tce_graph_launch",
                "tce_graph_destroy", "tce_graph_group"} | set(_lib.DEBUG_SIGNATURES)


class Launch:
    __slots__ = ("idx", "name", "stream", "tick", "clock", "reads", "writes", "site")

    def __repr__(self):
        return f"#{self.idx} {self.name} on stream {self.stream:#x} at {self.site}"


class Recorder:

    def __init__(self):
        self.launches = []
        self.clock = {}
        self.events = {}
        self.edges = 0
        self.host_syncs = 0

    def _clk(self, s):
        c = self.clock.get(int(s))
        if c is None:
            c = self.clock[int(s)] = dict(getattr(self, "_future", {}))
        return c

    def launch(self, name, stream, reads, writes, site):
        s = int(stream or 0)
        c = self._clk(s)
        c[s] = c.get(s, 0) + 1
        L = Launch()
        L.idx, L.name, L.stream, L.tick, L.clock = len(self.launches), name, s, c[s], dict(c)
        L.reads, L.writes, L.site = union(*reads), union(*writes), site
        self.launches.append(L)

    def record_event(self, ev, stream):
        self.events[id(ev)] = (ev, dict(self._clk(stream)))

    @staticmethod
    def _merge(c, snap):
        for k, v in snap.items():
            if v > c.get(k, 0):
                c[k] = v

    def wait_event(self, ev, stream):
        ent = self.events.get(id(ev))
        if ent is None:
            return
        self._merge(self._clk(stream), ent[1])
        self.edges += 1

    def host_sync(self, snap=None):
        if snap is None:
            snap = {}
            for c in self.clock.values():
                self._merge(snap, c)
        snap = dict(snap)
        self._future = getattr(self, "_future", {})
        self._merge(self._future, snap)
        for s in list(self.clock):
            self._merge(self.clock[s], snap)
        self.host_syncs += 1

    @staticmethod
    def ordered(a, b):
        return b.clock.get(a.stream, 0) >= a.tick

    def analyse(self, max_report=20):
        L = self.launches
        conflicts, pairs = [], 0
        by_stream = {}
        for x in L:
            by_stream.setdefault(x.stream, []).append(x)
        for j, b in enumerate(L):
            for s, lst in by_stream.items():
                if s == b.stream:
                    continue
                seen = b.clock.get(s, 0)
                for a in lst:
                    if a.idx >= b.idx:
                        break
                    if a.tick <= seen:
                        continue
                    pairs += 1
# ... 100 lines not shown
```

tce-rvos_amd/model.py:

```python
import os
import types
import math
from collections import OrderedDict
from typing import List, Optional

import torch
from torch import nn

from . import ops
from .config import ModelConfig, config_from_args, index_buffers, param_shapes
from .weights import synth_tensor

ACT_RELU, ACT_GELU = ops.ACT_RELU, ops.ACT_GELU
RES_ADD, RES_MUL = ops.RES_ADD, ops.RES_MUL


class NestedTensor(object):

    def __init__(self, tensors, mask: Optional[torch.Tensor]):
        self.tensors = tensors
        self.mask = mask

    def to(self, device):
        nt = NestedTensor(self.tensors.to(device), self.mask.to(device) if self.mask is not None else None)
# ... 394 lines not shown
        key = (T, H0, W0, valid)
        c = self._shape_cache.get(key)
        if c is not None:
            return c
        cfg, w = self.cfg, self._packed
        Hp, Wp = (H0 + 3) // 4, (W0 + 3) // 4
        sizes = [(Hp, Wp)]
        for _ in range(3):
            h, ww = sizes[-1]
            sizes.append(((h + 1) // 2, (ww + 1) // 2))
        h5, w5 = sizes[3]
        lvl_sizes = [sizes[1], sizes[2], sizes[3], ((h5 + 2 - 3) // 2 + 1, (w5 + 2 - 3) // 2 + 1)]
        S = sum(h * ww for h, ww in lvl_sizes)
        starts = [0]
        for h, ww in lvl_sizes[:-1]:
            starts.append(starts[-1] + h * ww)
        F = cfg.hidden_dim // 2
        c = dict(sizes=sizes, lvl_sizes=lvl_sizes, S=S, starts=starts)

        def nvalid(n_out, n_in, v_in):
            if v_in >= n_in:
                return n_out
            src = torch.clamp(torch.floor(torch.arange(n_out, dtype=torch.float32) *
                                          torch.tensor(float(n_in) / float(n_out), dtype=torch.float32)).long(), max=n_in - 1)
            return int((src < v_in).sum())

        Hv, Wv = valid if valid is not None else (H0, W0)
        sizes_v = [(nvalid(h, H0, Hv), nvalid(ww, W0, Wv)) for (h, ww) in sizes]
        lvl_v = [(nvalid(h, H0, Hv), nvalid(ww, W0, Wv)) for (h, ww) in lvl_sizes]
        if valid is not None and any(a < 1 or b < 1 for a, b in sizes_v + lvl_v):
            raise NotImplementedError("padded clip whose valid region vanishes at a pyramid level")
        c["lvl_valid"] = lvl_v if valid is not None else None
        c["pos"] = [ops.pos_sine2d(1, h, ww, F, device, valid=v) for (h, ww), v in zip(sizes, sizes_v)]
        lp = torch.empty(S, cfg.hidden_dim, dtype=torch.float32, device=device)
        for l, (h, ww) in enumerate(lvl_sizes):
            ops.pos_sine2d(1, h, ww, F, device, add=w["transformer.level_embed"][l], out=lp[starts[l]:starts[l] + h * ww],
                           valid=lvl_v[l])
        c["lvl_pos"] = lp
        refs = []
        for (h, ww), (hv, wv) in zip(lvl_sizes, lvl_v):
            ry, rx = torch.meshgrid(torch.linspace(0.5, h - 0.5, h, dtype=torch.float32),
                                    torch.linspace(0.5, ww - 0.5, ww, dtype=torch.float32), indexing="ij")
            if valid is None:
                refs.append(torch.stack((rx.reshape(-1) / ww, ry.reshape(-1) / h), -1))
            else:
                vr_w, vr_h = torch.tensor(float(wv)) / ww, torch.tensor(float(hv)) / h
                refs.append(torch.stack((rx.reshape(-1) / (vr_w * ww), ry.reshape(-1) / (vr_h * h)), -1))
        c["enc_ref"] = torch.cat(refs, 0).to(device).contiguous()
        red, kmask = {}, {}
        for stage, sr in ((1, 8), (2, 4), (3, 2), (4, 1)):
            h, ww = sizes[stage - 1]
            hv, wv = sizes_v[stage - 1]
            if sr > 1:
                nh_, nw_ = int(h * 1.0 / sr), int(ww * 1.0 / sr)
                red[stage] = (nh_, nw_, ops.resize_nearest(c["pos"][stage - 1], 1, h, ww, nh_, nw_, cfg.hidden_dim))
                h, ww, hv, wv = nh_, nw_, nvalid(nh_, h, hv), nvalid(nw_, ww, wv)
            if valid is not None:
                m = torch.ones(h, ww, dtype=torch.uint8)
                m[:hv, :wv] = 0
                kmask[stage] = m.reshape(-1).repeat(T).to(device).contiguous()
        c["red"] = red
        c["kmask"] = kmask
        torch.cuda.current_stream(device).synchronize()
        self._shape_cache[key] = c
        return c

    def _text_pos(self, L, device):
        key = ("text_pos", L)
        tp = self._shape_cache.get(key)
        if tp is None:
            x = torch.arange(1, L + 1, dtype=torch.float32)
            x = x / (x[-1:] + 1e-6) * (2 * math.pi)
            dim_t = torch.arange(self.cfg.hidden_dim, dtype=torch.float32)
            dim_t = 10000.0 ** (2 * torch.div(dim_t, 2, rounding_mode="trunc") / self.cfg.hidden_dim)
            px = x[:, None] / dim_t
            tp = torch.stack((px[:, 0::2].sin(), px[:, 1::2].cos()), dim=2).flatten(1).to(device).contiguous()
            self._shape_cache[key] = tp
        return tp

    @staticmethod
    def _conv3_ws_bytes(T, H0, W0, strides):
        return 4 * max(ops.conv3x3_split_ws_floats(T * (-(-H0 // s)) * (-(-W0 // s))) for s in strides)

    def _arena_bytes(self, T, H0, W0):
        tok0 = T * ((H0 + 3) // 4) * ((W0 + 3) // 4)
        return self.arena_bytes or int(tok0 * 4 * (2048 * 2.2 + 256 * 24) + (256 << 20) + self._conv3_ws_bytes(T, H0, W0, (4, 8)))

    def _get_arena(self, T, H0, W0, device, slot=0):
        need = self._arena_bytes(T, H0, W0)
        ar = self._arenas.get(slot)
        if ar is None or ar.buf.numel() < need or ar.device != torch.device(device):
            ar = self._arenas[slot] = ops.Arena(device, need)
        return ar

    @torch.no_grad()
    def forward(self, samples, captions, targets, slot=0):
        if not isinstance(samples, NestedTensor) and not (hasattr(samples, "tensors") and hasattr(samples, "mask")):
            if len(samples) == 1:
                vids, mask = samples[0][None], None
            else:
                samples = nested_tensor_from_videos_list(samples)
                vids, mask = samples.tensors, samples.mask
        else:
            vids, mask = samples.tensors, samples.mask
        if isinstance(captions, (list, tuple)):
            if not isinstance(captions[0], str):
                raise ValueError("Please mask sure the caption is a list of string")
            b = len(captions)
        else:
            b = captions.shape[0]
        if vids.dim() == 4:
            vids = vids[None]
        if b != 1 or vids.shape[0] != 1:
            raise NotImplementedError("one clip per forward (B = 1): the reference mixes clips inside a batch "
                                      "(FTF token attention, IQT) so batching changes results; shard clips instead")
        select = int(targets[0]["valid_indices"]) if "valid_indices" in targets[0] else None
        if select is not None and not 0 <= select < vids.shape[1]:
            raise IndexError(f"valid_indices {select} outside the clip's {vids.shape[1]} frames")
        if not vids.is_cuda:
            raise RuntimeError("inputs must be on the GPU: this path has no CPU implementation")
        frames = vids[0].to(torch.float32).contiguous()
        valid = self._valid_region(samples, mask, frames)
        size = targets[0]["size"]
        img_h, img_w = float(size[0]), float(size[1])
        ids, att, ids_host = self._tokenise(captions, frames.device)
        self._ensure_packed()
        ops.range_poll(frames.device)
        cached = self._text_lookup(ids, ids_host, frames.device)
        if cached is not None:
            out = self.forward_features(frames, cached[0], cached[1], img_h, img_w, slot=slot, valid_hw=valid, select=select)
        else:
            ids = ids.to(frames.device)
            key = ("clip", tuple(frames.shape), tuple(ids.shape), img_h, img_w, self.training, int(slot), self._stamp, valid, select)
            if not self._want_graph(key):
                out = self._run(frames, lambda alloc: self._text_plan().forward(ids, alloc), img_h, img_w, None, slot, valid=valid,
                                select=select)
            else:
                ent = self._graphs.get(key)
                if ent is None:
                    st = (frames.clone(), ids.clone())

                    def text_fn(alloc):
                        return self._text_plan().forward(st[1], alloc)

                    ent = self._capture(key, st, lambda res: self._run(st[0], text_fn, img_h, img_w, res, valid=valid, select=select),
                                        frames, slot)
                if ent is None:
                    out = self._run(frames, lambda alloc: self._text_plan().forward(ids, alloc), img_h, img_w, None, slot,
                                    valid=valid, select=select)
                else:
                    out = self._replay(key, ent, (frames, ids))
        ops.range_snapshot_async(frames.device)
        return self._tag_diagnostics(out)

    def _pad_id(self):
        return int(getattr(getattr(self.text_encoder, "config", None), "pad_token_id", 1) or 1)

    def _group_text(self, ids, ragged):
        if not ragged:
            return lambda alloc: self._text_plan().forward(ids, alloc)
        pad_id = self._pad_id()

        def text(alloc):
            rag = ops.caption_lens(ids, pad_id, alloc, self.cfg.hidden_dim)
            hid, pooled = self._text_plan().forward(ids, alloc, lens=rag[0])
            return hid, pooled, rag
        return text

    @torch.no_grad()
# ... 113 lines not shown
            return False
        if key in self._graphs:
            return True
        n = self._sightings.get(key, 0)
        self._sightings[key] = n + 1
        self._sightings.move_to_end(key)
        while len(self._sightings) > 256:
            self._sightings.popitem(last=False)
        if n < self.graph_after:
            return False
        if len(_ALL_GRAPHS) >= GRAPH_BUDGET and not (GRAPH_OWN_EXEC and os.environ.get("TCE_KEEP_GRAPHS", "0") != "1"):
            global _BUDGET_WARNED
            if not _BUDGET_WARNED:
                _BUDGET_WARNED = True
                import warnings
                warnings.warn(f"tce_rvos_amd: the process's hipGraph capture budget ({GRAPH_BUDGET}, TCE_GRAPH_BUDGET) is spent: "
                              f"shapes that are not cached now run as eager launches (same results, ~15 % slower per clip); "
                              f"model.graph_state() reports this", RuntimeWarning, stacklevel=3)
            return False
        return True

    @staticmethod
    def graph_state():
        return graph_state()

    def _text_lookup(self, ids, ids_host=None, device=None):
        if self.text_cache_size <= 0:
            return None
        key = tuple(int(v) for v in (ids if ids_host is None else ids_host).reshape(-1).tolist())
        ent = self._text_cache.get(key)
        if ent is None:
            ids = ids.to(device) if device is not None else ids
            hid, pooled = self._text_plan().forward(
                ids, lambda *shape: torch.empty(*shape, dtype=torch.float32, device=ids.device))
            ent = (hid, pooled)
            self._text_cache[key] = ent
            while len(self._text_cache) > self.text_cache_size:
                self._text_cache.popitem(last=False)
        else:
            self._text_cache.move_to_end(key)
        return ent

    def _tokenise(self, captions, device):
        if isinstance(captions, (list, tuple)):
            if isinstance(self.tokenizer, SyntheticTokenizer):
                ids, att = self.tokenizer(list(captions))
            else:
                tok = self.tokenizer.batch_encode_plus(list(captions), padding="longest", return_tensors="pt")
                ids, att = tok["input_ids"], tok["attention_mask"]
            if bool((att != 1).any()):
                raise NotImplementedError("padded captions (B > 1) are not supported")
        else:
            ids, att = captions, None
        return ids, att, (None if ids.is_cuda else ids)

    def _text_plan(self):
        if self._text is None:
            from .text_encoder import TextPlan
            self._text = TextPlan(self.text_encoder)
        return self._text

    def text_encoder_reference(self, ids, att=None):
        att = torch.ones_like(ids) if att is None else att
        enc = self.text_encoder(input_ids=ids, attention_mask=att)
        return enc.last_hidden_state.float(), enc.pooler_output.float()

    def _run(self, frames, text, img_h, img_w, res, slot=0, valid=None, groups=1, shared=False, select=None):
        from .pipeline import run_clip
        T, _, H0, W0 = frames.shape
        if res is None:
            return run_clip(self, frames, text, img_h, img_w, self._get_arena(T * (groups if shared else 1), H0, W0, frames.device, slot),
                            valid=valid, groups=groups, shared=shared, select=select)
        arena, side_arena, side_stream, arena2, stream2, arena3, stream3, arena4, stream4 = res
        return run_clip(self, frames, text, img_h, img_w, arena, side_arena, side_stream, clone_outputs=False, valid=valid,
                        groups=groups, shared=shared, select=select,
                        fork2=(arena2, stream2) if os.environ.get("TCE_FORK2", "1") != "0" else None,
                        fork3=((arena3, stream3), (arena4, stream4)) if os.environ.get("TCE_FORK3", "1") != "0" else None)

    def _branch_resources(self, like, slot=0):
        T, _, H0, W0 = like.shape
        tok0 = T * ((H0 + 3) // 4) * ((W0 + 3) // 4)
        st = _side_streams(like.device, slot)
        return (ops.Arena(like.device, self._arena_bytes(T, H0, W0)),
                ops.Arena(like.device, T * self._tokens_per_frame(H0, W0) * 256 * 4 * 4 + (32 << 20)),
                st[0],
                ops.Arena(like.device, int(tok0 * 4 * (2048 * 1.1 + 256 * 4)) + (64 << 20)),
                st[1],
                ops.Arena(like.device, max(int(tok0 / 64 * 4 * (2048 + 256 * 12)) + int(tok0 / 16 * 4 * 256 * 8),
                                           int(tok0 / 4 * 4 * 256 * 5)) + (64 << 20) + self._conv3_ws_bytes(T, H0, W0, (16, 32))),
                st[2],
                ops.Arena(like.device, int(tok0 / 16 * 4 * (2048 * 1.1 + 256 * 12)) + (64 << 20)),
                st[3])

    @torch.no_grad()
    def hazard_check(self, frames, ids, img_hw=None, valid=None, slot=0, dry=False, groups=1, shared=False, ragged=False):
        from . import hazard
        frames = frames.to(torch.float32).contiguous()
        T, _, H0, W0 = frames.shape
        img_h, img_w = (float(H0), float(W0)) if img_hw is None else (float(img_hw[0]), float(img_hw[1]))
        self._ensure_packed()
        res = self._branch_resources(types.SimpleNamespace(shape=(T * (groups if shared else 1), 3, H0, W0), device=frames.device), slot)
        st = (frames.clone(), ids.to(frames.device).clone())
        run = lambda: self._run(st[0], self._group_text(st[1], ragged), img_h, img_w, res, valid=valid, shared=shared,
                                groups=groups)
        main = torch.cuda.Stream(device=frames.device)
        main.wait_stream(torch.cuda.current_stream())
        with torch.cuda.stream(main):
            if not dry:
                run()
            torch.cuda.synchronize()
            with hazard.recording(dry=dry) as rec:
                run()
            torch.cuda.synchronize()
        torch.cuda.current_stream().wait_stream(main)
        return rec.analyse()

    def _capture(self, key, statics, fn, like, slot=0):
        res = self._branch_resources(like, slot)
        try:
            fn(res)
        except MemoryError as e:
            import warnings
            torch.cuda.synchronize()
            self._nograph.add(key)
            warnings.warn(f"tce_rvos_amd: graph capture of {key[:2]} skipped ({e}); this shape runs eagerly", RuntimeWarning)
            return None
        torch.cuda.synchronize()
        keep = os.environ.get("TCE_KEEP_GRAPHS", "0") == "1"
        own = GRAPH_OWN_EXEC and not keep
        graph = torch.cuda.CUDAGraph(keep_graph=True) if (keep or own) else torch.cuda.CUDAGraph()
        with torch.cuda.graph(graph, capture_error_mode="thread_local"):
            out = fn(res)
        if own:
            import ctypes as C
            from ._lib import lib
            raw = (C.c_void_p * 1)(int(graph.raw_cuda_graph()))
            ex = C.c_void_p()
            if lib().tce_graph_group(raw, 1, C.byref(ex)) == 0 and ex.value:
                del graph
                graph = _OwnedExec(ex)
            else:
                own = False
                graph.instantiate()
        elif keep:
            graph.instantiate()
        if not own:
            _ALL_GRAPHS.append(graph)
        try:
            plan = ops.CopyPlan(_flat_outputs(out)) if os.environ.get("TCE_COPYPLAN", "1") != "0" else None
        except ValueError:
            plan = None
        ent = (graph, statics, out, res, sum(r.buf.numel() for r in res if isinstance(r, ops.Arena)), plan)
        self._graphs[key] = ent
        while len(self._graphs) > 1 and (len(self._graphs) > self.max_graphs or
                                         sum(e[4] for e in self._graphs.values()) > self.max_graph_bytes):
            torch.cuda.synchronize()
            _, old = self._graphs.popitem(last=False)
            if isinstance(old[0], _OwnedExec):
                old[0].destroy()
        return ent

    @staticmethod
    def _tokens_per_frame(H0, W0):
        h, w = (H0 + 3) // 4, (W0 + 3) // 4
        n = 0
        for _ in range(3):
            h, w = (h + 1) // 2, (w + 1) // 2
# ... 139 lines not shown
```

tce-rvos_amd/ops.py:

```python
import ctypes as C

import os
import threading

import torch

from ._lib import GemmArgs, check, lib

ACT_NONE, ACT_RELU, ACT_GELU, ACT_RELU_AFTER_RES = 0, 1, 2, 3
RES_NONE, RES_ADD, RES_MUL = 0, 1, 2


class Arena:

    ALIGN = 256
    FLAGS = 1 << 14

    def __init__(self, device, nbytes):
        self.device = torch.device(device)
        self.buf = torch.empty(int(nbytes), dtype=torch.uint8, device=self.device)
        self.off = 0
        self.peak = 0
        self.flags = torch.zeros(self.FLAGS, dtype=torch.int32, device=self.device)
        self.flag_off = 0
# ... 1068 lines not shown


XATTN_FFN_CHAIN = os.environ.get("TCE_XATTN_FFN_CHAIN", "0") != "0"


def ffn_pack_chain(w1, b1, w2):
    _chk(w1, "w1")
    _chk(w2, "w2")
    Hd, Cn = w1.shape
    nbytes = lib().tce_ffn_packed_bytes(Cn, Hd)
    if Cn != 256 or nbytes < 0 or tuple(w2.shape) != (Cn, Hd):
        raise ValueError(f"ffn_pack_chain: unsupported shape C={Cn} hidden={Hd}")
    out = torch.empty(nbytes, dtype=torch.uint8, device=w1.device)
    check(lib().tce_ffn_pack_chain_f32(w1.contiguous().data_ptr(), b1.contiguous().data_ptr() if b1 is not None else None,
                                       w2.contiguous().data_ptr(), out.data_ptr(), Cn, Hd, _stream()), "tce_ffn_pack_chain_f32")
    return out


def xattn_fused(x, pk, bo, M, out, a2=None, lda2=256, a2_rows=0, res=None, res_mode=RES_ADD, ln_out=None, eps_out=1e-5,
                batch=1, sX=0, sRes=0, sOut=0, ldx=256, ldo=256, ldres=256, group=32, per_batch_weights=False, w_div=1, ffn=None):
    from ._lib import XattnArgs, XattnFfnArgs
    q = XattnArgs()
    q.x, q.packed, q.bo, q.out = x.data_ptr(), pk.data_ptr(), bo.data_ptr(), out.data_ptr()
    q.M, q.batch, q.res_mode, q.eps_out, q.group = M, batch, res_mode, eps_out, group
    q.sW = pk.stride(0) if (per_batch_weights and pk.dim() == 2) else 0
    q.w_div = max(1, int(w_div))
    q.ldx, q.ldo, q.ldres, q.lda2 = ldx, ldo, ldres, lda2
    q.sX, q.sRes, q.sOut = sX, sRes, sOut
    if a2 is not None:
        q.a2, q.a2_rows = a2.data_ptr(), a2_rows
    if res is not None:
        q.res = res.data_ptr()
    if ln_out is not None:
        q.g_out, q.be_out = ln_out[0].data_ptr(), ln_out[1].data_ptr()

    fq = None
    if ffn is not None:
        pk2, b2, hidden, ln2, mid, s_mid = ffn
        fq = XattnFfnArgs()
        fq.packed, fq.b2, fq.mid, fq.ldmid, fq.sMid, fq.hidden, fq.act = pk2.data_ptr(), b2.data_ptr(), mid.data_ptr(), 256, s_mid, hidden, 1
        if ln2 is not None:
            fq.g_out, fq.be_out, fq.eps_out = ln2[0].data_ptr(), ln2[1].data_ptr(), 1e-5

    def go():
        if fq is not None:
            check(lib().tce_xattn_ffn_fused_f32(C.byref(q), C.byref(fq), _stream()), "tce_xattn_ffn_fused_f32")
        else:
            check(lib().tce_xattn_fused_f32(C.byref(q), _stream()), "tce_xattn_fused_f32")
    if GEMM_PROFILE is None:
        go()
        return out
    e0, e1 = torch.cuda.Event(enable_timing=True), torch.cuda.Event(enable_timing=True)
    e0.record()
    go()
    e1.record()
    if fq is not None:
        GEMM_PROFILE.append(("xattn+ffn(ffn_fused_kernel<256,4,3|4,1>", False, 4.0 * M * 256 * (8 * group + hidden) * batch, e0, e1))
    else:
        GEMM_PROFILE.append(("xattn(ffn_fused_kernel<256,4,3|4>", False, 4.0 * M * 256 * 8 * group * batch, e0, e1))
    return out


FEWROW_MAX_ROWS = int(os.environ.get("TCE_FEWROW_MAX_ROWS", 128))
FR_NONE, FR_RELU, FR_SIGMOID, FR_GELU = 0, 1, 2, 3


def fewrow_linear(x, R, K, segs, ldx=None, a2=None, lda2=0, a2_rows=0, res=None, ldres=0, ln_in=None, eps_in=1e-5, xn_out=None):
    from ._lib import FewRowArgs
    q = FewRowArgs()
    if ln_in is not None:
        q.g_in, q.be_in, q.eps_in = ln_in[0].data_ptr(), ln_in[1].data_ptr(), eps_in
        if xn_out is not None:
            q.xn_out, q.ldxn = xn_out.data_ptr(), (xn_out.stride(0) if xn_out.dim() == 2 else K)
    q.x, q.ldx, q.R, q.K, q.nseg = x.data_ptr(), (K if ldx is None else ldx), R, K, len(segs)
    if a2 is not None:
        q.a2, q.lda2, q.a2_rows = a2.data_ptr(), lda2, a2_rows
    if res is not None:
        q.res, q.ldres = res.data_ptr(), ldres
    for i, (W, b, out, N, ldo, use_a2, act) in enumerate(segs):
        sg = q.seg[i]
        sg.W, sg.bias, sg.out = W.data_ptr(), (b.data_ptr() if b is not None else None), out.data_ptr()
        sg.N, sg.ldw, sg.ldo, sg.use_a2, sg.act = N, (W.stride(0) if W.dim() == 2 else K), ldo, 1 if use_a2 else 0, act
    check(lib().tce_fewrow_linear_f32(C.byref(q), _stream()), "tce_fewrow_linear_f32")
```

tce-rvos_amd/pipeline.py:

```python
import os

import torch

from . import ops
from .ops import ACT_GELU, ACT_RELU, ACT_RELU_AFTER_RES, RES_ADD, RES_MUL, gemm_ex

D = 256
NH = 8
FFN_FUSED_MIN_ROWS = int(__import__("os").environ.get("TCE_FFN_FUSED_MIN_ROWS", 16000))
SWIN_FUSED_MIN_TOKENS = int(os.environ.get("TCE_SWIN_FUSED_MIN_TOKENS", 2000))


def _proj_res_ln(x, wt, bias, resid, M, norm_w, norm_b):
    pk = ops.rowlin_lookup(wt, D, D) if M >= FFN_FUSED_MIN_ROWS else None
    if pk is not None:
        ops.rowlin(x, pk, resid, M, D, D, D, D, bias=bias, res=resid, ldres=D, res_mode=RES_ADD, ln_out=(norm_w, norm_b))
        return
    gemm_ex(x, wt, resid, M, D, D, D, D, D, bias=bias, res=resid, ldres=D, res_mode=RES_ADD)
    ops.layernorm(resid, norm_w, norm_b, 1e-5, out=resid)


def _lin(A, x, M, K, w, b, N, **kw):
    out = A(M, N)
    gemm_ex(x, w, out, M, N, K, K, K, N, bias=b, **kw)
# ... 538 lines not shown
        else:
            r = _lin(A, qpos, Q, D, w["transformer.reference_points.weight"], w["transformer.reference_points.bias"], 2)
            r = ops.sigmoid(r, out=A(Q, 2))
        init_ref = ops.tile(r, T, out=A(T * Q, 2))
        tgt = A(T * Q, D)
        for g_ in range(G):
            ops.tile(sent[g_], Tc * Q, out=tgt[g_ * Tc * Q:(g_ + 1) * Tc * Q])
        ref, ref_dim = init_ref, 2
        for lid in range(0 if "decoder" not in ABLATE else nl, nl):
            lp = f"transformer.decoder.layers.{lid}."
            m0 = dar.mark()
            pre = lp + "self_attn."
            prev, tgt = tgt, hs[lid]
            qk = A(T * Q, 2 * D)
            if few(T * Q, "dec"):
                v = A(T * Q, D)
                FR(prev, T * Q, D, [(w[pre + "qk.w"], w[pre + "qk.b"], qk, 2 * D, 2 * D, True, ops.FR_NONE),
                                    (w[pre + "v.w"], w[pre + "v.b"], v, D, D, False, ops.FR_NONE)], a2=qpos, lda2=D, a2_rows=Q)
            else:
                gemm_ex(prev, w[pre + "qk.w"], qk, Q, 2 * D, D, D, D, 2 * D, bias=w[pre + "qk.b"], a2=qpos, lda2=D, batch=T,
                        sA=Q * D, sA2=0, sC=Q * 2 * D)
                v = _lin(A, prev, T * Q, D, w[pre + "v.w"], w[pre + "v.b"], D)
            att = A(T * Q, D)
            if cfg.qtrans:
                for g_ in range(G):
                    r0 = g_ * Tc * Q
                    ops.mha_core(qk[r0:], qk[r0:, D:], v[r0:], Q, NH, Tc, Tc, Q * 2 * D, Q * 2 * D, Q * D, 2 * D, 2 * D, D, att[r0:],
                                 Q * D, D)
            else:
                ops.mha_core(qk, qk[:, D:], v, T, NH, Q, Q, 2 * D, 2 * D, D, Q * 2 * D, Q * 2 * D, Q * D, att, D, Q * D)
            if few(T * Q, "dec"):
                FR(att, T * Q, D, [(w[pre + "out_proj.weight"], w[pre + "out_proj.bias"], tgt, D, D, False, ops.FR_NONE)],
                   res=prev, ldres=D)
            else:
                gemm_ex(att, w[pre + "out_proj.weight"], tgt, T * Q, D, D, D, D, D, bias=w[pre + "out_proj.bias"], res=prev,
                        ldres=D, res_mode=RES_ADD)
            ln_(tgt, lp + "norm2")
            msda(lp + "cross_attn.", tgt, T * Q, Q, qpos, True, memory, ref, ref_dim, True, tgt, ar=dar, norm=lp + "norm1",
                 group="decoder")
            ffn(tgt, T * Q, lp, ar=dar, norm=lp + "norm3", group="decoder")
            if cfg.with_box_refine:
                bp = f"bbox_embed.{lid}.layers."
                t1, t2 = A(T * Q, D), A(T * Q, D)
                if few(T * Q, "dec"):
                    t3 = A(T * Q, 4)
                    segs = [(w[bp + "0.weight"], w[bp + "0.bias"], t1, D, D, False, ops.FR_RELU),
                            (w[f"class_embed.{lid}.weight"], w[f"class_embed.{lid}.bias"], logits[lid], cfg.num_classes,
                             cfg.num_classes, False, ops.FR_NONE)]
                    if vis is not None:
                        segs.append((w[f"visible_embed.{lid}.weight"], w[f"visible_embed.{lid}.bias"], vis[lid], 1, 1, False, ops.FR_NONE))
                    FR(tgt, T * Q, D, segs)
                    logits_done[lid] = True
                    FR(t1, T * Q, D, [(w[bp + "1.weight"], w[bp + "1.bias"], t2, D, D, False, ops.FR_RELU)])
                    FR(t2, T * Q, D, [(w[bp + "2.weight"], w[bp + "2.bias"], t3, 4, 4, False, ops.FR_NONE)])
                else:
                    gemm_ex(tgt, w[bp + "0.weight"], t1, T * Q, D, D, D, D, D, bias=w[bp + "0.bias"], act=ACT_RELU)
                    gemm_ex(t1, w[bp + "1.weight"], t2, T * Q, D, D, D, D, D, bias=w[bp + "1.bias"], act=ACT_RELU)
                    t3 = _lin(A, t2, T * Q, D, w[bp + "2.weight"], w[bp + "2.bias"], 4)
                ops.box_refine(t3, ref, out=inter_ref[lid])
                ref, ref_dim = inter_ref[lid], 4
            dar.release(m0)

        for lvl in range(nl):
            if logits_done[lvl]:
                continue
            ci = lvl if cfg.with_box_refine else 0
            gemm_ex(hs[lvl], w[f"class_embed.{ci}.weight"], logits[lvl], T * Q, cfg.num_classes, D, D, D, cfg.num_classes,
                    bias=w[f"class_embed.{ci}.bias"])
            if vis is not None:
                gemm_ex(hs[lvl], w[f"visible_embed.{ci}.weight"], vis[lvl], T * Q, 1, D, D, D, 1, bias=w[f"visible_embed.{ci}.bias"])
        if cfg.with_box_refine:
            return hs, inter_ref, inter_ref, 4, logits, vis
        refs2 = ops.tile(init_ref, nl, out=A(nl, T * Q, 2))
        bp = "bbox_embed.0.layers."
        t1 = A(nl * T * Q, D)
        gemm_ex(hs, w[bp + "0.weight"], t1, nl * T * Q, D, D, D, D, D, bias=w[bp + "0.bias"], act=ACT_RELU)
        t2 = A(nl * T * Q, D)
        gemm_ex(t1, w[bp + "1.weight"], t2, nl * T * Q, D, D, D, D, D, bias=w[bp + "1.bias"], act=ACT_RELU)
        t3 = _lin(A, t2, nl * T * Q, D, w[bp + "2.weight"], w[bp + "2.bias"], 4)
        ops.box_refine(t3, refs2, out=inter_ref)
        return hs, inter_ref, refs2, 2, logits, vis

    npar = cfg.num_gen_params
    dec_fork = _Fork(side_stream if side_arena is not None else None)
    with dec_fork, model.arith("decoder"):
        hs, boxes, mask_refs, ref_ld, logits, vis = decoder_branch()
        tap("dec.hs", hs)
        dA = dar.alloc
        c1 = dA(nl * T * Q, D)
        c2 = dA(nl * T * Q, D)
        if few(nl * T * Q, "dec"):
            params = dA(nl * T * Q, npar)
            FR(hs, nl * T * Q, D, [(w["controller.layers.0.weight"], w["controller.layers.0.bias"], c1, D, D, False, ops.FR_RELU)])
            FR(c1, nl * T * Q, D, [(w["controller.layers.1.weight"], w["controller.layers.1.bias"], c2, D, D, False, ops.FR_RELU)])
            FR(c2, nl * T * Q, D, [(w["controller.layers.2.weight"], w["controller.layers.2.bias"], params, npar, npar, False,
                                    ops.FR_NONE)])
        else:
            gemm_ex(hs, w["controller.layers.0.weight"], c1, nl * T * Q, D, D, D, D, D, bias=w["controller.layers.0.bias"],
                    act=ACT_RELU)
            gemm_ex(c1, w["controller.layers.1.weight"], c2, nl * T * Q, D, D, D, D, D, bias=w["controller.layers.1.bias"],
                    act=ACT_RELU)
            params = _lin(dA, c2, nl * T * Q, D, w["controller.layers.2.weight"], w["controller.layers.2.bias"], npar)
        w0f = dA(T, nl * Q * 8, cfg.mask_dim)
        tail = dA(nl, T * Q, 112)
        ops.mask_pack(params, nl, T, Q, cfg.mask_dim, w0f, tail)
        contrast = None
        if cfg.contrastive:
            contrast = dA(T)
            ops.contrastive(memory, sent, T, S, D, Tc, contrast, dA(T * 32 * D))

    _stage("decoder fork")
    while pending_norm0:
        pending_norm0.pop()()
    mask_feats = _pixel_decoder(model, ar, sc, feats, memory, vl_sites, T, L, ffn, ln_, lat1=lat1, par=fork3, G=G)
    dec_fork.join()

    _stage("pixel decoder")
    h4, w4 = sizes[0]
    m0 = ar.mark()
    gmat = A(T, h4 * w4, nl * Q * 8)
    with model.arith("mask_head"):
        ops.gemm_batched(mask_feats.view(T, h4 * w4, cfg.mask_dim), w0f, gmat)
    masks = A(nl, T, Q, h4, w4)
    ops.mask_tail(gmat, tail, mask_refs, ref_ld, masks, nl, T, Q, h4, w4, img_h, img_w, 4)

    _stage("mask head (+ decoder join)")
    K = cfg.num_classes
    keep = (lambda t: t.clone()) if clone_outputs else (lambda t: t)
    out = {
        "pred_logits": keep(logits[-1].reshape(1, T, Q, K)),
        "pred_boxes": keep(boxes[-1].reshape(1, T, Q, 4)),
        "pred_masks": keep(masks[-1].reshape(1, T, Q, h4, w4)),
    }
    if vis is not None:
        out["pred_visible"] = keep(vis[-1].reshape(1, T, Q, 1))
    if contrast is not None:
        out["contrastive"] = keep(contrast.reshape(1, T))
    if cfg.aux_loss:
        out["aux_outputs"] = [{"pred_logits": keep(logits[i].reshape(1, T, Q, K)),
                               "pred_boxes": keep(boxes[i].reshape(1, T, Q, 4)),
                               "pred_masks": keep(masks[i].reshape(1, T, Q, h4, w4))} for i in range(nl - 1)]
        if vis is not None:
            for i in range(nl - 1):
                out["aux_outputs"][i]["pred_visible"] = keep(vis[i].reshape(1, T, Q, 1))
    if not model.training:
        out["reference_points"] = keep(mask_refs[-2].reshape(1, T, Q, ref_ld)[..., :2])
    out["memory"] = keep(memory.reshape(T, S, D))
    if taps:
        out["taps"] = [{k_: keep(v_) for k_, v_ in taps.items()}]
    ar.release(m0)
    return out


def _swin_backbone(model, frames, ar, sizes, on_stage=None, G=1, rep=1):
    cfg, w = model.cfg, model._packed
    A = ar.alloc
    T = frames.shape[0]
    b = "backbone.0.body."
    C = cfg.embed_dim
    (H, W) = sizes[0]
    x = A(T * H * W, C)
    with model.arith("backbone.merge"):
        ops.patch_embed(frames, w[b + ("patch_embed.proj.weight:2d" if cfg.video else "patch_embed.proj.weight")],
                        w[b + "patch_embed.proj.bias"],
                        w[b + "patch_embed.norm.weight"], w[b + "patch_embed.norm.bias"], out=x)
    feats = []
    for i, depth in enumerate(cfg.depths):
        H, W = sizes[i]
        ntok = T * H * W
        nH = cfg.num_heads[i]
        out_i = A(rep * ntok, C) if (rep > 1 or not cfg.video) else None
        x_next = None
        if i < len(cfg.depths) - 1:
            H2, W2 = sizes[i + 1]
            x_next = A(T * H2 * W2, 2 * C)
        hid = int(C * cfg.mlp_ratio)
        for j in range(depth if f"swin{i}" not in ABLATE else 0):
            p = f"{b}layers.{i}.blocks.{j}."
            m0 = ar.mark()
            pk_attn = None
            if ops.SWIN_FUSED and not cfg.video and ntok >= SWIN_FUSED_MIN_TOKENS:
                pk_attn = w.get(p + "attn:pk:" + model.mode_of("backbone.attn"))
            if pk_attn is not None:
                with model.arith("backbone.attn"):
                    ops.swin_attn_fused(x, pk_attn, w[p + "attn.qkv.bias"], w[p + "attn.proj.bias"],
                                        w[p + "attn.relative_position_bias_table"], w[p + "norm1.weight"], w[p + "norm1.bias"],
                                        T, H, W, C, 0 if j % 2 == 0 else cfg.window_size // 2)
            xn = A(ntok, C)
            if pk_attn is None:
                with model.arith("backbone.attn"):
                    qkv = A(ntok, 3 * C)
                    pk = ops.rowlin_lookup(w[p + "attn.qkv.weight"], 3 * C, C) \
                        if ((C <= 128 and ntok >= 32768) or (C == 384 and 2048 <= ntok <= ops.ROWLIN384_MAX_ROWS)) else None
                    if pk is not None:
                        ops.rowlin(x, pk, qkv, ntok, 3 * C, C, C, 3 * C, bias=w[p + "attn.qkv.bias"],
                                   ln_in=(w[p + "norm1.weight"], w[p + "norm1.bias"]))
                    else:
                        ops.layernorm(x, w[p + "norm1.weight"], w[p + "norm1.bias"], out=xn)
                        gemm_ex(xn, w[p + "attn.qkv.weight"], qkv, ntok, 3 * C, C, C, C, 3 * C, bias=w[p + "attn.qkv.bias"])
                    if cfg.video:
                        nc = ntok // G
                        for g_ in range(G):
                            ops.window_attn3d(qkv[g_ * nc:(g_ + 1) * nc], w[p + "attn.qkv.bias"],
                                              w[p + "attn.relative_position_bias_table"], T // G, H, W, C, nH, j % 2 == 1,
                                              out=xn[g_ * nc:(g_ + 1) * nc])
# ... 100 lines not shown
    A = arx.alloc
    h, ww = sizes[stage - 1]
    hw = h * ww
    pos = sc["pos"][stage - 1]
    vis = A(T * hw, D)
    with model.arith("pixel.conv"):
        if stage > 1:
            l = stage - 2
            gemm_ex(memory[starts[l]:], w[f"{pd}adapter_{stage}.weight"], vis, hw, D, D, D, D, D, batch=T, sA=S * D,
                    sC=hw * D)
        else:
            c0 = cfg.num_channels[0]
            gemm_ex(feats[0], w[f"{pd}adapter_1.weight"], vis, T * hw, D, c0, c0, c0, D)
    m1 = arx.mark()
    tgt = ops.groupnorm_cl(vis, w[f"{pd}adapter_{stage}.norm.weight"], w[f"{pd}adapter_{stage}.norm.bias"], T, hw, D, 8,
                           out=vis, alloc=A)
    arx.release(m1)
    if not cfg.vlblock:
        return tgt
    bp = f"{pd}cross_attn_{stage}."
    pre = bp + "self_attn."
    red = sc["red"].get(stage)
    normed = False
    with model.arith("pixel.attn"):
        m1 = arx.mark()
        if red is not None:
            nh_, nw_, pos_low = red
            n_low = T * nh_ * nw_
            x_low = ops.resize_nearest(tgt, T, h, ww, nh_, nw_, D, alloc=A)
            qk = A(n_low, 2 * D)
            gemm_ex(x_low, w[pre + "qk.w"], qk, nh_ * nw_, 2 * D, D, D, D, 2 * D, bias=w[pre + "qk.b"], a2=pos_low,
                    lda2=D, batch=T, sA=nh_ * nw_ * D, sA2=0, sC=nh_ * nw_ * 2 * D)
            v = _lin(A, x_low, n_low, D, w[pre + "v.w"], w[pre + "v.b"], D)
            att = A(n_low, D)
            nc = n_low // G
            ops.mha_core(qk, qk[:, D:], v, G, NH, nc, nc, 2 * D, 2 * D, D, nc * 2 * D, nc * 2 * D, nc * D, att, D, nc * D, alloc=A,
                         kmask=sc["kmask"].get(stage))
            o_low = _lin(A, att, n_low, D, w[pre + "out_proj.weight"], w[pre + "out_proj.bias"], D)
            ops.resize_bilinear(o_low, T, nh_, nw_, h, ww, D, add=tgt, out=tgt, ln=(w[bp + "norm1.weight"], w[bp + "norm1.bias"]))
            normed = True
        else:
            n = T * hw
            qk = A(n, 2 * D)
            gemm_ex(tgt, w[pre + "qk.w"], qk, hw, 2 * D, D, D, D, 2 * D, bias=w[pre + "qk.b"], a2=pos, lda2=D,
                    batch=T, sA=hw * D, sA2=0, sC=hw * 2 * D)
            v = _lin(A, tgt, n, D, w[pre + "v.w"], w[pre + "v.b"], D)
            att = A(n, D)
            nc = n // G
            ops.mha_core(qk, qk[:, D:], v, G, NH, nc, nc, 2 * D, 2 * D, D, nc * 2 * D, nc * 2 * D, nc * D, att, D, nc * D, alloc=A,
                         kmask=sc["kmask"].get(stage))
            gemm_ex(att, w[pre + "out_proj.weight"], tgt, n, D, D, D, D, D, bias=w[pre + "out_proj.bias"], res=tgt,
                    ldres=D, res_mode=RES_ADD)
        arx.release(m1)
    if not normed:
        ln_(tgt, bp + "norm1")
    pre = bp + "multihead_attn."
    with model.arith("pixel.xattn"):
        m1 = arx.mark()
        tk, tv, pk, tkm = vl_sites[stage]
        Mc = (T // G) * hw
        chained = None
        if pk is not None:
            chained = ffn.chain(bp, "pixel.ffn", T * hw, bp + "norm3", A, Mc * D)
            ops.xattn_fused(tgt, pk, w[pre + "out_proj.bias"], Mc, tgt, a2=pos, a2_rows=hw,
                            ln_out=(w[bp + "norm2.weight"], w[bp + "norm2.bias"]), batch=G, sX=Mc * D, sOut=Mc * D,
                            per_batch_weights=G > 1, ffn=chained)
        else:
            q = A(T * hw, D)
            gemm_ex(tgt, w[pre + "q.w"], q, hw, D, D, D, D, D, bias=w[pre + "q.b"], a2=pos, lda2=D, batch=T, sA=hw * D,
                    sA2=0, sC=hw * D)
            att = A(T * hw, D)
            ops.mha_core(q, tk, tv, G, NH, Mc, L, D, D, D, Mc * D, L * D, L * D, att, D, Mc * D, kmask=tkm)
            _proj_res_ln(att, w[pre + "out_proj.weight"], w[pre + "out_proj.bias"], tgt, T * hw, w[bp + "norm2.weight"],
                         w[bp + "norm2.bias"])
        arx.release(m1)
    if chained is None:
        ffn(tgt, T * hw, bp, norm=bp + "norm3", ar=arx, group="pixel.ffn")
    if _TAP_FN is not None:
        _TAP_FN(f"vl{stage}", tgt)
    return tgt



def _pixel_decoder(model, ar, sc, feats, memory, vl_sites, T, L, ffn, ln_, lat1=None, par=None, G=1):
    cfg, w = model.cfg, model._packed
    A = ar.alloc
    sizes = sc["sizes"]
    pd = "pixel_decoder."

    pending = {}

    def merge_conv(tgt, stage, y, y_hw, arx, y_new):
        h, ww = sizes[stage - 1]
        if y is not None:
            prev = pending.pop(id(y), None)
            if prev is not None:
                ops.groupnorm_up_add(y, w[f"{pd}layer_{prev}.norm.weight"], w[f"{pd}layer_{prev}.norm.bias"], T, y_hw[0], y_hw[1], h, ww,
                                     D, 8, add=tgt, out=tgt, relu=True, alloc=arx.alloc)
            else:
                ops.resize_nearest(y, T, y_hw[0], y_hw[1], h, ww, D, add=tgt, out=tgt)
        if ops.GN_UP_FUSE and stage > 1:
            with model.arith("pixel.conv"):
                ops.conv2d_cl(tgt, w[f"{pd}layer_{stage}.weight:cl"], T, h, ww, D, 3, 3, 1, 1, out=y_new, alloc=arx.alloc)
            pending[id(y_new)] = stage
            return
        with model.arith("pixel.conv"):
            conv, _, _ = ops.conv2d_cl(tgt, w[f"{pd}layer_{stage}.weight:cl"], T, h, ww, D, 3, 3, 1, 1, alloc=arx.alloc)
        ops.groupnorm_cl(conv, w[f"{pd}layer_{stage}.norm.weight"], w[f"{pd}layer_{stage}.norm.bias"], T, h * ww, D, 8,
                         relu=True, out=y_new, alloc=arx.alloc)

    y = None
    y_hw = None
    stages = (4, 3, 2, 1)
    if par is not None and par[0][1] is not None and par[1][1] is not None:
        (ar3, st3), (ar4, st4) = par
        ar3.reset()
        ar4.reset()
        fk_l3 = _Fork(st4)
        with fk_l3:
            tgt3 = _lateral(model, sc, feats, memory, vl_sites, T, L, ffn, ln_, 3, ar4, G)
        fk_c = _Fork(st3)
        with fk_c:
            (h4, w4), (h3, w3) = sizes[3], sizes[2]
            y4, y3 = ar3.alloc(T * h4 * w4, D), ar3.alloc(T * h3 * w3, D)
            tgt4 = _lateral(model, sc, feats, memory, vl_sites, T, L, ffn, ln_, 4, ar3, G)
            merge_conv(tgt4, 4, None, None, ar3, y4)
            fk_l3.join()
            merge_conv(tgt3, 3, y4, (h4, w4), ar3, y3)
        h, ww = sizes[1]
        y2 = A(T * h * ww, D)
        m0 = ar.mark()
        tgt2 = _lateral(model, sc, feats, memory, vl_sites, T, L, ffn, ln_, 2, ar, G)
        fk_c.join()
        merge_conv(tgt2, 2, y3, (h3, w3), ar, y2)
        ar.release(m0)
        y, y_hw = y2, (h, ww)
        stages = (1,)
    for stage in stages:
        h, ww = sizes[stage - 1]
        hw = h * ww
        y_new = A(T * hw, D)
        m0 = ar.mark()
        if stage == 1 and lat1 is not None:
            lat1[0].join()
            tgt = lat1[1]
        else:
            tgt = _lateral(model, sc, feats, memory, vl_sites, T, L, ffn, ln_, stage, ar, G)
        merge_conv(tgt, stage, y, y_hw, ar, y_new)
        ar.release(m0)
        y, y_hw = y_new, (h, ww)
    h, ww = sizes[0]
    with model.arith("pixel.conv"):
        out_final, _, _ = ops.conv2d_cl(y, w[pd + "mask_features.weight:cl"], T, h, ww, D, 3, 3, 1, 1,
                                        bias=w[pd + "mask_features.bias"], alloc=A)
    return out_final
```

Before: 173.3 clips/s.

## Fold mask-head dynamic weights into the mask_features 3x3 conv

Instead of running the 256->256 mask_features 3x3 conv and then a per-frame batched GEMM with the dynamic mask weights (nl*Q*8 outputs), the per-frame dynamic weights are multiplied into the conv weights and bias up front. A single per-frame 3x3 conv then produces the mask logits directly, with N = nl*Q*8 output channels. The conv kernel is generalised to fewer output tiles and per-frame weight and bias offsets. This removes one full-resolution conv output write and read plus a GEMM launch, at the cost of a per-clip fold/pack kernel and changed rounding order under split fp16.

```diff
diff --git a/include/tce_rvos.h b/include/tce_rvos.h
--- a/include/tce_rvos.h
+++ b/include/tce_rvos.h
@@ -202,6 +202,11 @@
 int32_t tce_conv3x3_split_kstep(int32_t pieces, int32_t s);
 int tce_conv3x3_split_f32(const float* x, int64_t ldx, const void* packed, const float* bias, float* out, int64_t ldo, int32_t T,
                           int32_t H, int32_t W, int32_t Cin, int32_t N, float* ws, int64_t ws_floats, tceStream stream);
+int64_t tce_conv3x3_frames_packed_bytes(int32_t Cin, int32_t N);
+int tce_conv3x3_fold_pack_f32(const float* w0f, const float* w, const float* b, void* packed, float* bias_out, int32_t F, int32_t N,
+                              int32_t Cin, tceStream stream);
+int tce_conv3x3_frames_f32(const float* x, int64_t ldx, const void* packed, const float* bias, float* out, int64_t ldo, int32_t T,
+                           int32_t H, int32_t W, int32_t Cin, int32_t N, tceStream stream);
 
 typedef struct {
   const float* x;
diff --git a/tce-rvos_amd/_lib.py b/tce-rvos_amd/_lib.py
--- a/tce-rvos_amd/_lib.py
+++ b/tce-rvos_amd/_lib.py
@@ -135,6 +135,9 @@
     "tce_conv3x3_split_pieces": (i32, [i32, i32, i32]),
     "tce_conv3x3_split_kstep": (i32, [i32, i32]),
     "tce_conv3x3_split_f32": (i32, [c_f, i64, c_f, c_f, c_f, i64, i32, i32, i32, i32, i32, c_f, i64, c_f]),
+    "tce_conv3x3_frames_packed_bytes": (i64, [i32, i32]),
+    "tce_conv3x3_fold_pack_f32": (i32, [c_f, c_f, c_f, c_f, c_f, i32, i32, i32, c_f]),
+    "tce_conv3x3_frames_f32": (i32, [c_f, i64, c_f, c_f, c_f, i64, i32, i32, i32, i32, i32, c_f]),
     "tce_fewrow_linear_f32": (i32, [C.POINTER(FewRowArgs), c_f]),
     "tce_thin_linear_splits": (i32, [i32, i32, i32]),
     "tce_thin_partials_f32": (i32, [c_f, i64, i32, c_f, i32, c_f, i64, c_f, i32, i32, i32, c_f]),
diff --git a/tce-rvos_amd/build.py b/tce-rvos_amd/build.py
--- a/tce-rvos_amd/build.py
+++ b/tce-rvos_amd/build.py
@@ -10,7 +10,7 @@
 LIBDIR = os.path.join(HERE, "lib")
 LIB = os.path.join(LIBDIR, "libtce_rvos.so")
 SOURCES = ["gemm_f16x3_big_256_split.hip", "gemm_f16x3_big_256_single.hip", "gemm_f16x3_big_128_split.hip", "gemm_f16x3_big_128_single.hip",
-           "chain_ffn.hip", "chain_rowlin.hip", "gemm_f16x3_big.hip", "gemm_f16x3_small.hip", "gemm.hip", "attn.hip", "misc.hip", "norm.hip", "msda.hip",
+           "chain_ffn.hip", "chain_rowlin.hip", "chain_conv3.hip", "gemm_f16x3_big.hip", "gemm_f16x3_small.hip", "gemm.hip", "attn.hip", "misc.hip", "norm.hip", "msda.hip",
            "text.hip", "resnet.hip", "frontend.hip", "fewrow.hip", "swinattn.hip", "thin.hip", "capi.hip"]
 HIPCC = os.environ.get("HIPCC", "/opt/rocm/bin/hipcc")
 FLAGS = ["--offload-arch=gfx950", "-O3", "-fPIC", "-std=c++17", "-Wall", "-Wno-unused-function"] + \
diff --git a/tce-rvos_amd/csrc/chain.hip b/tce-rvos_amd/csrc/chain.hip
--- a/tce-rvos_amd/csrc/chain.hip
+++ b/tce-rvos_amd/csrc/chain.hip
@@ -1102,7 +1102,11 @@
   int m_off;
   int nb, pieces;
   float* ws;
+  int hw, sb;
+  long long sw;
 };
+
+__host__ __device__ constexpr int conv3x3_stage_pieces(const int nt) { return 4 * ((nt + 1) / 2); }
 
 constexpr int CONV_ITERS = 12;
 __host__ __device__ constexpr int conv3x3_piece_iter(const int pieces, const int s) { return s * CONV_ITERS / pieces; }
@@ -1124,11 +1128,13 @@
   }
 }
 
-template <int CIN, bool SINGLE, int WAVES = 4, bool SPLIT = false>
+template <int CIN, bool SINGLE, int WAVES = 4, bool SPLIT = false, int NT = 8, bool FRAMES = false>
 __global__ void __launch_bounds__(64 * WAVES, WAVES / 4) conv3x3_kernel(const ConvArgs p) {
-  constexpr int NTL = 8;
-  constexpr int PW = 16 / WAVES;
-  constexpr int STAGE = 2 * NTL * PIECE;
+  constexpr int NTL = NT;
+  constexpr int SP = conv3x3_stage_pieces(NT);
+  constexpr int PW = SP / WAVES;
+  constexpr int STAGE = SP * PIECE;
+  static_assert(NT >= 1 && NT <= 8 && SP % WAVES == 0 && PW <= 4, "stage pieces divide over the waves");
   constexpr int R = 4;
   constexpr int XS = WAVES == 4 ? 6 : 4, LX = XS + 1;
   constexpr int NW = WAVES == 4 ? CONV_PAD_STAGES - 2 : 3, LW = NW + 2;
@@ -1139,9 +1145,9 @@
   constexpr int KS = BODY * ITERS;
   static_assert(CIN % 64 == 0, "channel chunks come in groups of four");
   static_assert(BODY % R == 0 && BODY % XS == 0 && BODY % NW == 0 && LX >= LW, "ring positions are compile-time");
-  static_assert(WAVES * WT_BYTES <= R * STAGE, "the epilogue's staging tiles alias the ring");
-  static_assert(!SPLIT || (ITERS == CONV_ITERS && WAVES == 4 && !SINGLE), "split pieces: CIN = 256, 128-pixel workgroups, split fp16");
-  __shared__ __attribute__((aligned(16))) unsigned char smem[R * STAGE];
+  static_assert(!SPLIT || (ITERS == CONV_ITERS && WAVES == 4 && !SINGLE && NT == 8 && !FRAMES),
+                "split pieces: CIN = 256, N = 256, 128-pixel workgroups, split fp16");
+  __shared__ __attribute__((aligned(16))) unsigned char smem[R * STAGE > WAVES * WT_BYTES ? R * STAGE : WAVES * WT_BYTES];
 
   const int tid = threadIdx.x, lane = tid & 63;
   const int wave = __builtin_amdgcn_readfirstlane(tid >> 6);
@@ -1150,15 +1156,23 @@
   const int piece = SPLIT ? (int)blockIdx.x / p.nb : 0;
   const int i0 = SPLIT ? conv3x3_piece_iter(p.pieces, piece) : 0;
   const int i1 = SPLIT ? conv3x3_piece_iter(p.pieces, piece + 1) : ITERS;
-  const int m0 = p.m_off + blk * (32 * WAVES) + wave * 32;
+  int frame = 0, m0 = p.m_off + blk * (32 * WAVES) + wave * 32, mend = p.M;
+  if constexpr (FRAMES) {
+    const int nbf = (p.hw + 32 * WAVES - 1) / (32 * WAVES);
+    frame = blk / nbf;
+    m0 = frame * p.hw + (blk - frame * nbf) * (32 * WAVES) + wave * 32;
+    mend = min(p.M, (frame + 1) * p.hw);
+  }
+  const unsigned char* const wpk = FRAMES ? p.wpk + (long long)frame * p.sw : p.wpk;
+  const float* const bias = FRAMES && p.bias ? p.bias + (long long)frame * p.sb : p.bias;
 
   const int m = m0 + (lane & 31);
   const int px = m % p.W, py = (m / p.W) % p.H;
-  const float* const zeros = reinterpret_cast<const float*>(p.wpk + (long long)(KS + CONV_PAD_STAGES) * STAGE) + 8 * hf;
-  const float* const xme = p.x + (long long)min(m, p.M - 1) * p.ldx + 8 * hf;
+  const float* const zeros = reinterpret_cast<const float*>(wpk + (long long)(KS + CONV_PAD_STAGES) * STAGE) + 8 * hf;
+  const float* const xme = p.x + (long long)min(m, mend - 1) * p.ldx + 8 * hf;
   auto iter_ptrs = [&](const int it, const float* (&q)[3]) {
     const int dy = it / (CIN / 64) - 1, cq = it % (CIN / 64);
-    const bool row_ok = it < i1 && m < p.M && (unsigned)(py + dy) < (unsigned)p.H;
+    const bool row_ok = it < i1 && m < mend && (unsigned)(py + dy) < (unsigned)p.H;
 #pragma unroll
     for (int d = 0; d < 3; ++d) {
       const bool ok = row_ok && (unsigned)(px + d - 1) < (unsigned)p.W;
@@ -1166,18 +1180,11 @@
     }
   };
 
-  const float* wp = reinterpret_cast<const float*>(p.wpk + ((long long)i0 * BODY * STAGE) + (long long)(PW * wave) * PIECE + lane * 16);
+  const float* wp = reinterpret_cast<const float*>(wpk + ((long long)i0 * BODY * STAGE) + (long long)(PW * wave) * PIECE + lane * 16);
   unsigned char* const wdst = smem + (PW * wave) * PIECE + lane * 16;
   f32x4 wr[NW][PW];
   auto wload = [&](f32x4 (&dst)[PW]) {
-    if (!(CONV_ABL & 8)) {
-      gload16<0>(dst[0], wp);
-      gload16<PIECE>(dst[1], wp);
-      if constexpr (PW == 4) {
-        gload16<2 * PIECE>(dst[2], wp);
-        gload16<3 * PIECE>(dst[3], wp);
-      }
-    }
+    if (!(CONV_ABL & 8)) static_for<0, PW>([&](auto qc) { gload16<decltype(qc)::value * PIECE>(dst[decltype(qc)::value], wp); });
     wp += STAGE / 4;
   };
   auto wstore = [&](const f32x4 (&src)[PW], const int stage) {
@@ -1205,8 +1212,12 @@
                    : "+v"(xs[0]), "+v"(xs[1]), "+v"(ws[0]), "+v"(ws[1]), "+v"(ws[2]), "+v"(ws[3])
                    : "n"(N)
                    : "memory");
+    } else if constexpr (PW == 3) {
+      asm volatile("s_waitcnt vmcnt(%5)" : "+v"(xs[0]), "+v"(xs[1]), "+v"(ws[0]), "+v"(ws[1]), "+v"(ws[2]) : "n"(N) : "memory");
+    } else if constexpr (PW == 2) {
+      asm volatile("s_waitcnt vmcnt(%4)" : "+v"(xs[0]), "+v"(xs[1]), "+v"(ws[0]), "+v"(ws[1]) : "n"(N) : "memory");
     } else {
-      asm volatile("s_waitcnt vmcnt(%4)" : "+v"(xs[0]), "+v"(xs[1]), "+v"(ws[0]), "+v"(ws[1]) : "n"(N) : "memory");
+      asm volatile("s_waitcnt vmcnt(%3)" : "+v"(xs[0]), "+v"(xs[1]), "+v"(ws[0]) : "n"(N) : "memory");
     }
   };
   using nfl = std::integral_constant<int, INFLIGHT>;
@@ -1239,64 +1250,73 @@
     const unsigned char* const st = smem + lane * 16;
     fh[0] = *reinterpret_cast<const h16x8*>(st);
     fl[0] = *reinterpret_cast<const h16x8*>(st + PIECE);
-    fh[1] = *reinterpret_cast<const h16x8*>(st + 2 * PIECE);
-    fl[1] = *reinterpret_cast<const h16x8*>(st + 3 * PIECE);
-  }
+    if constexpr (NT > 1) {
+      fh[1] = *reinterpret_cast<const h16x8*>(st + 2 * PIECE);
+      fl[1] = *reinterpret_cast<const h16x8*>(st + 3 * PIECE);
+    }
+  }
+  constexpr int NPRE = NT > 2 ? NT - 2 : 0;
 
   for (int it = i0; it < i1; ++it) {
     static_for<0, BODY>([&](auto jc) {
       constexpr int j = decltype(jc)::value;
+      constexpr int g0 = j * NT;
       constexpr int nslot = (j + 1) % XS;
       const unsigned char* const st = smem + (j % R) * STAGE + lane * 16;
       unsigned nh[4], nl[4];
       auto tile = [&](auto tc) {
-        constexpr int t = decltype(tc)::value;
+        constexpr int t = decltype(tc)::value, f = (g0 + t) % 4;
 #if CONV_ABL & 4
-        const h16x8 k0 = fh[t % 4], k1 = fl[t % 4], k2 = bh, k3 = bl;
+        const h16x8 k0 = fh[f], k1 = fl[f], k2 = bh, k3 = bl;
         asm volatile("" : : "v"(k0), "v"(k1), "v"(k2), "v"(k3));
 #else
         if constexpr (!SINGLE) {
-          acc[t] = __builtin_amdgcn_mfma_f32_32x32x16_f16(fh[t % 4], bl, acc[t], 0, 0, 0);
-          acc[t] = __builtin_amdgcn_mfma_f32_32x32x16_f16(fl[t % 4], bh, acc[t], 0, 0, 0);
+          acc[t] = __builtin_amdgcn_mfma_f32_32x32x16_f16(fh[f], bl, acc[t], 0, 0, 0);
+          acc[t] = __builtin_amdgcn_mfma_f32_32x32x16_f16(fl[f], bh, acc[t], 0, 0, 0);
         }
-        acc[t] = __builtin_amdgcn_mfma_f32_32x32x16_f16(fh[t % 4], bh, acc[t], 0, 0, 0);
+        acc[t] = __builtin_amdgcn_mfma_f32_32x32x16_f16(fh[f], bh, acc[t], 0, 0, 0);
 #endif
       };
-      static_for<0, 6>([&](auto tc) {
+      auto split = [&](auto tc) {
         constexpr int t = decltype(tc)::value;
-        fh[(t + 2) % 4] = *reinterpret_cast<const h16x8*>(st + (2 * t + 4) * PIECE);
-        fl[(t + 2) % 4] = *reinterpret_cast<const h16x8*>(st + (2 * t + 5) * PIECE);
+        const float a = xr[nslot][t >> 1][2 * (t & 1)], b = xr[nslot][t >> 1][2 * (t & 1) + 1];
+        if constexpr (SINGLE) {
+          nh[t] = __builtin_bit_cast(unsigned, fp16x2_t{(__fp16)a, (__fp16)b});
+          nl[t] = 0u;
+        } else {
+          const fp16x2_t h = __builtin_amdgcn_cvt_pkrtz(a, b);
+          nh[t] = __builtin_bit_cast(unsigned, h);
+          nl[t] = __builtin_bit_cast(unsigned, __builtin_amdgcn_cvt_pkrtz(a - (float)h[0], b - (float)h[1]));
+        }
+        asm volatile("" : "+v"(nh[t]), "+v"(nl[t]));
+      };
+      static_for<0, NPRE>([&](auto tc) {
+        constexpr int t = decltype(tc)::value, f = (g0 + t + 2) % 4;
+        fh[f] = *reinterpret_cast<const h16x8*>(st + (2 * t + 4) * PIECE);
+        fl[f] = *reinterpret_cast<const h16x8*>(st + (2 * t + 5) * PIECE);
         __builtin_amdgcn_sched_barrier(0);
         tile(tc);
-        if constexpr (t < 4) {
-          const float a = xr[nslot][t >> 1][2 * (t & 1)], b = xr[nslot][t >> 1][2 * (t & 1) + 1];
-          if constexpr (SINGLE) {
-            nh[t] = __builtin_bit_cast(unsigned, fp16x2_t{(__fp16)a, (__fp16)b});
-            nl[t] = 0u;
-          } else {
-            const fp16x2_t h = __builtin_amdgcn_cvt_pkrtz(a, b);
-            nh[t] = __builtin_bit_cast(unsigned, h);
-            nl[t] = __builtin_bit_cast(unsigned, __builtin_amdgcn_cvt_pkrtz(a - (float)h[0], b - (float)h[1]));
-          }
-          asm volatile("" : "+v"(nh[t]), "+v"(nl[t]));
-        }
+        if constexpr (t < 4) split(tc);
         __builtin_amdgcn_sched_barrier(0);
       });
+      static_for<(NPRE < 4 ? NPRE : 4), 4>([&](auto tc) { split(tc); });
       wait_loads(nfl{}, xr[(j + 2) % XS], wr[(j + 2) % NW]);
       wstore(wr[(j + 2) % NW], (j + 2) % R);
       if (!(CONV_ABL & 2)) __syncthreads();
       xload(std::integral_constant<int, j + LX>{}, xr[(j + LX) % XS]);
       wload(wr[(j + LW) % NW]);
       {
+        constexpr int f0 = (g0 + NT) % 4, f1 = (g0 + NT + 1) % 4;
         const unsigned char* const sn = smem + ((j + 1) % R) * STAGE + lane * 16;
-        fh[0] = *reinterpret_cast<const h16x8*>(sn);
-        fl[0] = *reinterpret_cast<const h16x8*>(sn + PIECE);
-        fh[1] = *reinterpret_cast<const h16x8*>(sn + 2 * PIECE);
-        fl[1] = *reinterpret_cast<const h16x8*>(sn + 3 * PIECE);
+        fh[f0] = *reinterpret_cast<const h16x8*>(sn);
+        fl[f0] = *reinterpret_cast<const h16x8*>(sn + PIECE);
+        if constexpr (NT > 1) {
+          fh[f1] = *reinterpret_cast<const h16x8*>(sn + 2 * PIECE);
+          fl[f1] = *reinterpret_cast<const h16x8*>(sn + 3 * PIECE);
+        }
       }
       __builtin_amdgcn_sched_barrier(0);
-      tile(std::integral_constant<int, 6>{});
-      tile(std::integral_constant<int, 7>{});
+      static_for<NPRE, NT>([&](auto tc) { tile(tc); });
       __builtin_amdgcn_sched_barrier(0);
       bh = __builtin_bit_cast(h16x8, u32x4{nh[0], nh[1], nh[2], nh[3]});
       bl = __builtin_bit_cast(h16x8, u32x4{nl[0], nl[1], nl[2], nl[3]});
@@ -1306,6 +1326,14 @@
     iter_ptrs(it + 2, nxt);
   }
   asm volatile("s_waitcnt vmcnt(0)" ::: "memory");
+  if constexpr (NT < 8) {
+#pragma unroll
+    for (int i = 0; i < XS; ++i) asm volatile("" : : "v"(xr[i][0]), "v"(xr[i][1]));
+#pragma unroll
+    for (int i = 0; i < NW; ++i)
+#pragma unroll
+      for (int q = 0; q < PW; ++q) asm volatile("" : : "v"(wr[i][q]));
+  }
   __syncthreads();
 
   float* const wt = reinterpret_cast<float*>(smem + wave * WT_BYTES);
@@ -1319,8 +1347,8 @@
   const ResTile none = {};
 #pragma unroll
   for (int t = 0; t < NTL; ++t) {
-    tile_bias_res<0>(acc[t], tile_bias_load(p.bias, 32 * t, lane), none, wt, lane);
-    tile_store(acc[t], p.out, p.ldo, m0, p.M, 32 * t, wt, lane, amax);
+    tile_bias_res<0>(acc[t], tile_bias_load(bias, 32 * t, lane), none, wt, lane);
+    tile_store(acc[t], p.out, p.ldo, m0, mend, 32 * t, wt, lane, amax);
   }
   tce_range_report(p.range_flag, amax);
 }
@@ -1366,6 +1394,83 @@
 
 inline bool conv3x3_shape_ok(int Cin, int N) { return Cin == 256 && N == 256; }
 inline long long conv3x3_units(int Cin) { return (long long)(9 * Cin / 16 + CONV_PAD_STAGES) * 16 * 64 + 128; }
+
+inline bool conv3x3_frames_shape_ok(int Cin, int N) { return Cin == 256 && N >= 32 && N <= 256 && N % 32 == 0; }
+inline long long conv3x3_frame_units(int N) { return (long long)(9 * 256 / 16 + CONV_PAD_STAGES) * conv3x3_stage_pieces(N / 32) * 64 + 128; }
+
+constexpr int FOLD_FILL = 4;
+__global__ void __launch_bounds__(256) conv3x3_fold_pack_kernel(const float* __restrict__ w0f, const float* __restrict__ w,
+                                                                const float* __restrict__ b, unsigned char* __restrict__ out,
+                                                                float* __restrict__ bias_out, const int N, const long long units,
+                                                                const int single) {
+  constexpr int C = 256, CIN = 256, KT = 9 * CIN, S = KT / 16;
+  const int NT = N / 32, SP = conv3x3_stage_pieces(NT), f = blockIdx.y, tid = threadIdx.x;
+  const float* const a = w0f + (long long)f * N * C;
+  u32x4* const o = reinterpret_cast<u32x4*>(out + (long long)f * units * 16);
+  const int ntile = NT * (KT / 128);
+  if ((int)blockIdx.x >= ntile) {
+    const int q = (int)blockIdx.x - ntile;
+    if (q == 0 && tid < N) {
+      float acc = 0.f;
+      if (b)
+        for (int c = 0; c < C; ++c) acc = fmaf(a[(long long)tid * C + c], b[c], acc);
+      bias_out[(long long)f * N + tid] = acc;
+    }
+    const long long npad = (NT & 1) ? (long long)S * 128 : 0, tail0 = (long long)S * SP * 64;
+    const long long nz = npad + (units - tail0);
+    for (long long e = (long long)q * 256 + tid; e < nz; e += FOLD_FILL * 256) {
+      const long long u = e < npad ? (((e >> 7) * SP + 2 * NT + ((e >> 6) & 1)) << 6) + (e & 63) : tail0 + (e - npad);
+      o[u] = u32x4{0u, 0u, 0u, 0u};
+    }
+    return;
+  }
+  const int nt = (int)blockIdx.x % NT, kt = (int)blockIdx.x / NT;
+  __shared__ float As[32][33];
+  __shared__ __attribute__((aligned(16))) float Bs[32][128];
+  const int tx = tid & 15, ty = tid >> 4;
+  float acc[2][8];
+#pragma unroll
+  for (int i = 0; i < 2; ++i)
+#pragma unroll
+    for (int e = 0; e < 8; ++e) acc[i][e] = 0.f;
+  for (int c0 = 0; c0 < C; c0 += 32) {
+    {
+      const int r = tid >> 3, q4 = tid & 7;
+      const f32x4 v = *reinterpret_cast<const f32x4*>(a + (long long)(32 * nt + r) * C + c0 + 4 * q4);
+#pragma unroll
+      for (int e = 0; e < 4; ++e) As[4 * q4 + e][r] = v[e];
+    }
+#pragma unroll
+    for (int i = 0; i < 4; ++i) {
+      const int c = (tid >> 5) + 8 * i, k4 = tid & 31;
+      *reinterpret_cast<f32x4*>(&Bs[c][4 * k4]) = *reinterpret_cast<const f32x4*>(w + (long long)(c0 + c) * KT + 128 * kt + 4 * k4);
+    }
+    __syncthreads();
+#pragma unroll 8
+    for (int c = 0; c < 32; ++c) {
+      const float a0 = As[c][2 * ty], a1 = As[c][2 * ty + 1];
+      const f32x4 b0 = *reinterpret_cast<const f32x4*>(&Bs[c][8 * tx]), b1 = *reinterpret_cast<const f32x4*>(&Bs[c][8 * tx + 4]);
+#pragma unroll
+      for (int e = 0; e < 4; ++e) {
+        acc[0][e] = fmaf(a0, b0[e], acc[0][e]);
+        acc[0][4 + e] = fmaf(a0, b1[e], acc[0][4 + e]);
+        acc[1][e] = fmaf(a1, b0[e], acc[1][e]);
+        acc[1][4 + e] = fmaf(a1, b1[e], acc[1][4 + e]);
+      }
+    }
+    __syncthreads();
+  }
+  const int k = 128 * kt + 8 * tx, tap = k / CIN, cin = k % CIN, dy = tap / 3, dx = tap % 3, cc = cin / 16, hf = (cin >> 3) & 1;
+  const long long s = 12 * (dy * (CIN / 64) + cc / 4) + 3 * (cc % 4) + dx;
+#pragma unroll
+  for (int i = 0; i < 2; ++i) {
+    const int n = 32 * nt + 2 * ty + i;
+    const HL h = split8(acc[i], single);
+    const long long u = ((s * SP + 2 * (n >> 5)) << 6) + 32 * hf + (n & 31);
+    o[u] = __builtin_bit_cast(u32x4, h.hi);
+    o[u + 64] = __builtin_bit_cast(u32x4, h.lo);
+  }
+}
 
 template <int NT>
 __global__ void __launch_bounds__(256) patch_embed_mfma_kernel(const float* __restrict__ frames, const float* __restrict__ w,
@@ -1454,7 +1559,7 @@
 #endif
 int tce_chain_rowlin_set_stamps(long long* dev_buf);
 
-#if TCE_CHAIN_PART != 2
+#if TCE_CHAIN_PART != 2 && TCE_CHAIN_PART != 3
 extern "C" int tce_debug_ffn_set_stamp_buffer(long long* dev_buf) {
 #if TCE_CHAIN_PART == 1
   if (tce_chain_rowlin_set_stamps(dev_buf) != 0) return -1;
@@ -1700,7 +1805,7 @@
 
 #endif
 
-#if TCE_CHAIN_PART != 1
+#if TCE_CHAIN_PART != 1 && TCE_CHAIN_PART != 3
 int tce_chain_rowlin_set_stamps(long long* dev_buf) {
   return hipMemcpyToSymbol(HIP_SYMBOL(g_ffn_stamps), &dev_buf, sizeof(dev_buf)) == hipSuccess ? 0 : -1;
 }
@@ -1757,7 +1862,7 @@
 
 #endif
 
-#if TCE_CHAIN_PART != 2
+#if TCE_CHAIN_PART != 2 && TCE_CHAIN_PART != 3
 extern "C" int64_t tce_conv3x3_packed_bytes(int32_t Cin, int32_t N) { return conv3x3_shape_ok(Cin, N) ? conv3x3_units(Cin) * 16 : -1; }
 
 extern "C" int tce_conv3x3_pack_f32(const float* w, void* packed, int32_t Cin, int32_t N, tceStream stream) {
@@ -1857,7 +1962,7 @@
   a.x = x; a.wpk = (const unsigned char*)packed; a.bias = bias; a.out = out;
   a.ldx = ldx; a.ldo = ldo; a.H = H; a.W = W; a.M = T * H * W;
   a.range_flag = tce_range_flag(); a.single = tce_gemm_single_pass();
-  a.m_off = 0; a.nb = 0; a.pieces = 1; a.ws = nullptr;
+  a.m_off = 0; a.nb = 0; a.pieces = 1; a.ws = nullptr; a.hw = 0; a.sb = 0; a.sw = 0;
   hipStream_t s = (hipStream_t)stream;
   const Conv3Plan pl = conv3x3_plan_for(a.M, split);
   if (pl.pieces > 1)
@@ -1904,3 +2009,57 @@
   return true;
 }
 #endif
+
+#if TCE_CHAIN_PART == 0 || TCE_CHAIN_PART == 3
+extern "C" int64_t tce_conv3x3_frames_packed_bytes(int32_t Cin, int32_t N) {
+  return conv3x3_frames_shape_ok(Cin, N) ? conv3x3_frame_units(N) * 16 : -1;
+}
+
+extern "C" int tce_conv3x3_fold_pack_f32(const float* w0f, const float* w, const float* b, void* packed, float* bias_out, int32_t F,
+                                         int32_t N, int32_t Cin, tceStream stream) {
+  TCE_CHECK_ARG(conv3x3_frames_shape_ok(Cin, N), "tce_conv3x3_fold_pack_f32: unsupported shape Cin=%d N=%d (256 -> 32k, k = 1..8)", Cin, N);
+  TCE_CHECK_ARG(w0f && w && packed && bias_out && F > 0 && tce_aligned16(w0f) && tce_aligned16(w) && tce_aligned16(packed),
+                "tce_conv3x3_fold_pack_f32: null / misaligned pointer or F < 1");
+  const long long units = conv3x3_frame_units(N);
+  hipLaunchKernelGGL(conv3x3_fold_pack_kernel, dim3(N / 32 * (9 * 256 / 128) + FOLD_FILL, F), dim3(256), 0, (hipStream_t)stream, w0f, w,
+                     b, (unsigned char*)packed, bias_out, N, units, tce_gemm_single_pass());
+  TCE_CHECK_LAUNCH("tce_conv3x3_fold_pack_f32");
+  return TCE_OK;
+}
+
+template <int NT>
+static void conv3x3_frames_go(const ConvArgs& a, const int nb, hipStream_t s) {
+  if (a.single) hipLaunchKernelGGL((conv3x3_kernel<256, true, 4, false, NT, true>), dim3(nb), dim3(256), 0, s, a);
+  else hipLaunchKernelGGL((conv3x3_kernel<256, false, 4, false, NT, true>), dim3(nb), dim3(256), 0, s, a);
+}
+
+extern "C" int tce_conv3x3_frames_f32(const float* x, int64_t ldx, const void* packed, const float* bias, float* out, int64_t ldo,
+                                      int32_t T, int32_t H, int32_t W, int32_t Cin, int32_t N, tceStream stream) {
+  const char* name = "tce_conv3x3_frames_f32";
+  TCE_CHECK_ARG(conv3x3_frames_shape_ok(Cin, N), "%s: unsupported shape Cin=%d N=%d (256 -> 32k, k = 1..8)", name, Cin, N);
+  TCE_CHECK_ARG(x && packed && out && T > 0 && H > 0 && W > 0 && (long long)T * H * W < (1ll << 31), "%s: null pointer or bad sizes", name);
+  TCE_CHECK_ARG(ldx >= Cin && ldx % 4 == 0 && ldo >= N && ldo % 4 == 0, "%s: bad row pitch", name);
+  TCE_CHECK_ARG(tce_aligned16(x) && tce_aligned16(out) && tce_aligned16(packed) && (!bias || tce_aligned16(bias)),
+                "%s: pointers must be 16-byte aligned", name);
+  ConvArgs a;
+  a.x = x; a.wpk = (const unsigned char*)packed; a.bias = bias; a.out = out;
+  a.ldx = ldx; a.ldo = ldo; a.H = H; a.W = W; a.M = T * H * W;
+  a.range_flag = tce_range_flag(); a.single = tce_gemm_single_pass();
+  a.m_off = 0; a.nb = 0; a.pieces = 1; a.ws = nullptr;
+  a.hw = H * W; a.sb = N; a.sw = conv3x3_frame_units(N) * 16;
+  const int nb = T * tce_cdiv(a.hw, 128);
+  hipStream_t s = (hipStream_t)stream;
+  switch (N / 32) {
+    case 1: conv3x3_frames_go<1>(a, nb, s); break;
+    case 2: conv3x3_frames_go<2>(a, nb, s); break;
+    case 3: conv3x3_frames_go<3>(a, nb, s); break;
+    case 4: conv3x3_frames_go<4>(a, nb, s); break;
+    case 5: conv3x3_frames_go<5>(a, nb, s); break;
+    case 6: conv3x3_frames_go<6>(a, nb, s); break;
+    case 7: conv3x3_frames_go<7>(a, nb, s); break;
+    default: conv3x3_frames_go<8>(a, nb, s); break;
+  }
+  TCE_CHECK_LAUNCH(name);
+  return TCE_OK;
+}
+#endif
diff --git a/tce-rvos_amd/csrc/chain_conv3.hip b/tce-rvos_amd/csrc/chain_conv3.hip
--- /dev/null
+++ b/tce-rvos_amd/csrc/chain_conv3.hip
@@ -0,0 +1,2 @@
+#define TCE_CHAIN_PART 3
+#include "chain.hip"
diff --git a/tce-rvos_amd/hazard.py b/tce-rvos_amd/hazard.py
--- a/tce-rvos_amd/hazard.py
+++ b/tce-rvos_amd/hazard.py
@@ -368,6 +368,13 @@
          dense(_p(a[3]), a[10] * F)],
         [strided(_p(a[4]), a[10] * F, (a[6] * a[7] * a[8], a[5] * F)),
          dense(_p(a[11]), _lib.lib_raw().tce_conv3x3_split_ws_floats(a[6] * a[7] * a[8], a[9], a[10]) * F)]),
+    "tce_conv3x3_fold_pack_f32": lambda a: (
+        [dense(_p(a[0]), a[5] * a[6] * 256 * F), dense(_p(a[1]), 256 * 9 * a[7] * F), dense(_p(a[2]), 256 * F)],
+        [dense(_p(a[3]), a[5] * _lib.lib_raw().tce_conv3x3_frames_packed_bytes(a[7], a[6])), dense(_p(a[4]), a[5] * a[6] * F)]),
+    "tce_conv3x3_frames_f32": lambda a: (
+        [strided(_p(a[0]), a[9] * F, (a[6] * a[7] * a[8], a[1] * F)),
+         dense(_p(a[2]), a[6] * _lib.lib_raw().tce_conv3x3_frames_packed_bytes(a[9], a[10])), dense(_p(a[3]), a[6] * a[10] * F)],
+        [strided(_p(a[4]), a[10] * F, (a[6] * a[7] * a[8], a[5] * F))]),
     "tce_fewrow_linear_f32": lambda a: _fewrow(_st(a[0])),
     "tce_thin_partials_f32": lambda a: (
         [(strided(_p(a[0]), a[10] * F, (a[8], a[1] * F)) if a[2] == 0 else dense(_p(a[0]), a[2] * a[8] * a[10] * F)),
@@ -399,7 +406,7 @@
 NOT_LAUNCHES = {"tce_abi_version", "tce_last_error", "tce_gemm_select_tile", "tce_gemm_select_tile_ex", "tce_set_gemm_mode", "tce_set_gemm_mode_thread",
                 "tce_get_gemm_mode", "tce_set_range_flag", "tce_groupnorm_nsplit", "tce_mha_ws_bytes", "tce_ffn_packed_bytes", "tce_ffn_split_ws_floats", "tce_ffn_split_counters",
                 "tce_rowlin_packed_bytes", "tce_conv3x3_packed_bytes", "tce_conv3x3_split_ws_floats",
-                "tce_conv3x3_split_pieces", "tce_conv3x3_split_kstep", "tce_swin_attn_packed_bytes", "tce_thin_linear_splits", "tce_graph_begin", "tce_graph_end", "tce_graph_launch",
+                "tce_conv3x3_split_pieces", "tce_conv3x3_split_kstep", "tce_conv3x3_frames_packed_bytes", "tce_swin_attn_packed_bytes", "tce_thin_linear_splits", "tce_graph_begin", "tce_graph_end", "tce_graph_launch",
                 "tce_graph_destroy", "tce_graph_group"} | set(_lib.DEBUG_SIGNATURES)
 
 
diff --git a/tce-rvos_amd/model.py b/tce-rvos_amd/model.py
--- a/tce-rvos_amd/model.py
+++ b/tce-rvos_amd/model.py
@@ -500,9 +500,13 @@
     def _conv3_ws_bytes(T, H0, W0, strides):
         return 4 * max(ops.conv3x3_split_ws_floats(T * (-(-H0 // s)) * (-(-W0 // s))) for s in strides)
 
+    def _mask_fold_bytes(self, T):
+        return ops.mask_fold_bytes(T, self.cfg.dec_layers * self.cfg.num_queries * 8) if ops.MASK_FOLD else 0
+
     def _arena_bytes(self, T, H0, W0):
         tok0 = T * ((H0 + 3) // 4) * ((W0 + 3) // 4)
-        return self.arena_bytes or int(tok0 * 4 * (2048 * 2.2 + 256 * 24) + (256 << 20) + self._conv3_ws_bytes(T, H0, W0, (4, 8)))
+        return self.arena_bytes or int(tok0 * 4 * (2048 * 2.2 + 256 * 24) + (256 << 20) + self._conv3_ws_bytes(T, H0, W0, (4, 8)) +
+                                       self._mask_fold_bytes(T))
 
     def _get_arena(self, T, H0, W0, device, slot=0):
         need = self._arena_bytes(T, H0, W0)
@@ -782,7 +786,7 @@
         tok0 = T * ((H0 + 3) // 4) * ((W0 + 3) // 4)
         st = _side_streams(like.device, slot)
         return (ops.Arena(like.device, self._arena_bytes(T, H0, W0)),
-                ops.Arena(like.device, T * self._tokens_per_frame(H0, W0) * 256 * 4 * 4 + (32 << 20)),
+                ops.Arena(like.device, T * self._tokens_per_frame(H0, W0) * 256 * 4 * 4 + (32 << 20) + self._mask_fold_bytes(T)),
                 st[0],
                 ops.Arena(like.device, int(tok0 * 4 * (2048 * 1.1 + 256 * 4)) + (64 << 20)),
                 st[1],
diff --git a/tce-rvos_amd/ops.py b/tce-rvos_amd/ops.py
--- a/tce-rvos_amd/ops.py
+++ b/tce-rvos_amd/ops.py
@@ -1174,3 +1174,58 @@
         sg.W, sg.bias, sg.out = W.data_ptr(), (b.data_ptr() if b is not None else None), out.data_ptr()
         sg.N, sg.ldw, sg.ldo, sg.use_a2, sg.act = N, (W.stride(0) if W.dim() == 2 else K), ldo, 1 if use_a2 else 0, act
     check(lib().tce_fewrow_linear_f32(C.byref(q), _stream()), "tce_fewrow_linear_f32")
+
+
+MASK_FOLD = os.environ.get("TCE_MASK_FOLD", "1") != "0"
+
+
+def mask_fold_route(conv_mode, head_mode, cin, nd, mask_dim, enabled=None):
+    if not (MASK_FOLD if enabled is None else enabled):
+        return "unfolded (TCE_MASK_FOLD=0)"
+    if conv_mode != "f16x3" or head_mode != "f16x3":
+        return f"unfolded (arithmetic {conv_mode}/{head_mode}: split fp16 only)"
+    if cin != 256 or mask_dim != 256:
+        return f"unfolded (Cin {cin}, mask_dim {mask_dim}: 256 only)"
+    if nd % 32 != 0 or not 32 <= nd <= 256:
+        return f"unfolded (Nd {nd}: a multiple of 32 up to 256 only)"
+    return "fold"
+
+
+def mask_fold_bytes(F, nd, cin=256):
+    pk = int(lib().tce_conv3x3_frames_packed_bytes(cin, nd))
+    if pk < 0:
+        return 0
+    return F * pk + 256 + F * nd * 4 + 256
+
+
+def conv3x3_fold_pack(w0f, w_cl, bias, alloc):
+    _chk(w0f, "w0f")
+    _chk(w_cl, "w")
+    F, nd, cm = w0f.shape
+    cin = w_cl.shape[1] // 9
+    nbytes = int(lib().tce_conv3x3_frames_packed_bytes(cin, nd))
+    if nbytes < 0 or cm != w_cl.shape[0] or not w0f.is_contiguous() or not w_cl.is_contiguous():
+        raise ValueError(f"conv3x3_fold_pack: unsupported shape w0f {tuple(w0f.shape)} w {tuple(w_cl.shape)}")
+    pk = alloc(F * nbytes, dtype=torch.uint8)
+    b_out = alloc(F, nd)
+    check(lib().tce_conv3x3_fold_pack_f32(w0f.data_ptr(), w_cl.data_ptr(), bias.data_ptr() if bias is not None else None, pk.data_ptr(),
+                                          b_out.data_ptr(), F, nd, cin, _stream()), "tce_conv3x3_fold_pack_f32")
+    return pk, b_out
+
+
+def conv3x3_frames(x, pk, bias, T, H, W, Cin, N, out):
+    _chk(x, "x")
+    _chk(out, "out")
+
+    def go():
+        check(lib().tce_conv3x3_frames_f32(x.data_ptr(), x.stride(0), pk.data_ptr(), bias.data_ptr() if bias is not None else None,
+                                           out.data_ptr(), out.stride(0), T, H, W, Cin, N, _stream()), "tce_conv3x3_frames_f32")
+    if GEMM_PROFILE is None:
+        go()
+        return out
+    e0, e1 = torch.cuda.Event(enable_timing=True), torch.cuda.Event(enable_timing=True)
+    e0.record()
+    go()
+    e1.record()
+    GEMM_PROFILE.append((f"conv3x3_frames<{N}", True, 2.0 * T * H * W * N * 9 * Cin, e0, e1))
+    return out
diff --git a/tce-rvos_amd/pipeline.py b/tce-rvos_amd/pipeline.py
--- a/tce-rvos_amd/pipeline.py
+++ b/tce-rvos_amd/pipeline.py
@@ -644,6 +644,8 @@
         return hs, inter_ref, refs2, 2, logits, vis
 
     npar = cfg.num_gen_params
+    model.mask_head_path = ops.mask_fold_route(model.mode_of("pixel.conv"), model.mode_of("mask_head"), D, nl * Q * 8, cfg.mask_dim)
+    fold = model.mask_head_path == "fold"
     dec_fork = _Fork(side_stream if side_arena is not None else None)
     with dec_fork, model.arith("decoder"):
         hs, boxes, mask_refs, ref_ld, logits, vis = decoder_branch()
@@ -666,6 +668,10 @@
         w0f = dA(T, nl * Q * 8, cfg.mask_dim)
         tail = dA(nl, T * Q, 112)
         ops.mask_pack(params, nl, T, Q, cfg.mask_dim, w0f, tail)
+        if fold:
+            with model.arith("pixel.conv"):
+                fold_pk = ops.conv3x3_fold_pack(w0f, w["pixel_decoder.mask_features.weight:cl"], w["pixel_decoder.mask_features.bias"],
+                                                dA)
         contrast = None
         if cfg.contrastive:
             contrast = dA(T)
@@ -674,15 +680,19 @@
     _stage("decoder fork")
     while pending_norm0:
         pending_norm0.pop()()
-    mask_feats = _pixel_decoder(model, ar, sc, feats, memory, vl_sites, T, L, ffn, ln_, lat1=lat1, par=fork3, G=G)
+    mask_feats = _pixel_decoder(model, ar, sc, feats, memory, vl_sites, T, L, ffn, ln_, lat1=lat1, par=fork3, G=G, mask_features=not fold)
     dec_fork.join()
 
     _stage("pixel decoder")
     h4, w4 = sizes[0]
     m0 = ar.mark()
     gmat = A(T, h4 * w4, nl * Q * 8)
-    with model.arith("mask_head"):
-        ops.gemm_batched(mask_feats.view(T, h4 * w4, cfg.mask_dim), w0f, gmat)
+    if fold:
+        with model.arith("pixel.conv"):
+            ops.conv3x3_frames(mask_feats, fold_pk[0], fold_pk[1], T, h4, w4, D, nl * Q * 8, gmat.view(T * h4 * w4, nl * Q * 8))
+    else:
+        with model.arith("mask_head"):
+            ops.gemm_batched(mask_feats.view(T, h4 * w4, cfg.mask_dim), w0f, gmat)
     masks = A(nl, T, Q, h4, w4)
     ops.mask_tail(gmat, tail, mask_refs, ref_ld, masks, nl, T, Q, h4, w4, img_h, img_w, 4)
 
@@ -949,7 +959,7 @@
 
 
 
-def _pixel_decoder(model, ar, sc, feats, memory, vl_sites, T, L, ffn, ln_, lat1=None, par=None, G=1):
+def _pixel_decoder(model, ar, sc, feats, memory, vl_sites, T, L, ffn, ln_, lat1=None, par=None, G=1, mask_features=True):
     cfg, w = model.cfg, model._packed
     A = ar.alloc
     sizes = sc["sizes"]
@@ -1016,6 +1026,8 @@
         merge_conv(tgt, stage, y, y_hw, ar, y_new)
         ar.release(m0)
         y, y_hw = y_new, (h, ww)
+    if not mask_features:
+        return y
     h, ww = sizes[0]
     with model.arith("pixel.conv"):
         out_final, _, _ = ops.conv2d_cl(y, w[pd + "mask_features.weight:cl"], T, h, ww, D, 3, 3, 1, 1,
```

Result: no change. 173.4 clips/s, median of 6 (+0.0%).
